# uoguelph-mlrg/Theano-MPI

Measured on NVIDIA H100. Metric: AlexNet-128b BSP seconds per 5120 images (train+comm, device-timed, max over ranks), lower is better.
Workload: dtype bf16; 1 GPU; model=AlexNet, global_batch=128, input=3x227x227, parallelism=dp1, rule=BSP, push_master=False, cuda_graph=True, overlap=True

## Files before the change

theanompi_b200/csrc/api.h:

```cpp
#pragma once
#include <cuda_runtime.h>
#include <stdint.h>
#include <tuple>
#include "common.cuh"

namespace tmpi {

constexpr int kMaxRanks = 8;
constexpr int kMaxCommBlocks = 1024;

struct CommCtx {
  void* arena[kMaxRanks];
  uint32_t* sig[kMaxRanks];
  uint32_t* epoch;
  void* mc_arena;
  int rank, world;
  long long spin_limit;
};

struct FusedArgs {
  CommCtx ctx;
  long long w_off, g_off, u_off, h_off, wire_off;
  const uint8_t* block_group;
  GroupTable tab;
  const float* lr_ptr;
  float mu;
  int nesterov;
  float inv_k;
  long long lo, hi;
  int wire16;
  int pre_reduced;
  int push_master = 1;
};

struct ReduceArgs {
  CommCtx ctx;
  long long src_off, dst_off, h_off;
  const uint8_t* block_group;
  GroupTable tab;
  float scale;
  long long lo, hi;
  int skip_local_groups;
};

void gemm_set_debug(int flags);
void gemm_set_bulk(int mask);
void gemm_rs_configure(int world, const void* const* peer_g , const void* local_g);
void gemm_rs_add_range(const void* c_lo, const void* c_hi, long long blo, long long per);
void gemm_rs_clear();
int gemm_plan_splits(int tiles, int num_kb, int sms);
int gemm_plan_tall(long long M, int nt, int out_bf16, int sms);
std::tuple<int, int, int> gemm_plan_conv(int kind, long long M, int N, int groups, int num_kb, int tall_ok, int sms);
void gemm(const void* A, const void* B, void* C, const float* bias, int M, int N, int K, long long lda, long long ldb, long long ldc,
          int a_mn, int b_mn, int out_bf16, int bias_mode, int relu, float alpha, int bn_hint, int splitk, int f32, cudaStream_t st,
          int accumulate = 0);
void gemm_sgd(const void* A, const void* B, void* W, void* U, void* H, const void* lr_ptr, float lr_mult, float wd, float mu, int nesterov,
              float inv_k, int M, int N, int K, long long lda, long long ldb, long long ldw, int f32, cudaStream_t st);

void conv_fprop(const void* x, const void* w, void* y, const float* bias, int N, int H, int W, int Ctot, int c_off, int Cg, int KH,
                int KW, int Ho, int Wo, int S, int P, int O, long long ldc, int relu, int dgrad, int f32, cudaStream_t st);
void conv_wgrad(const void* dy, const void* x, void* dw, int N, int H, int W, int Ctot, int c_off, int Cg, int KH, int KW, int Ho,
                int Wo, int S, int P, int O, long long ldy, int accumulate, int f32, cudaStream_t st);
void conv_fprop2(const void* x, const void* w0, const void* w1, void* y0, void* y1, const float* bias0, const float* bias1, int N, int H,
                 int W, int Ctot, int c_off0, int c_off1, int Cg, int KH, int KW, int Ho, int Wo, int S, int P, int O, long long ldc,
                 int relu, int dgrad, int f32, cudaStream_t st);
void conv_wgrad2(const void* dy0, const void* dy1, const void* x, void* dw0, void* dw1, int N, int H, int W, int Ctot, int c_off0,
                 int c_off1, int Cg, int KH, int KW, int Ho, int Wo, int S, int P, int O, long long ldy, int accumulate, int f32,
                 cudaStream_t st);

void space_to_depth(const void* x, void* y, int N, int H, int W, int C, int S, int Hs, int Ws, int Cp, int P, int f32, cudaStream_t st);
void s2d_filter(const void* src, void* dst, int O, int KH, int KW, int C, int S, int KHs, int KWs, int Cp, int dir, int f32, cudaStream_t st);
void lrn_fwd(const void* x, void* y, long long rows, int C, int n, float k, float alpha, float beta, int f32, cudaStream_t st);
void lrn_bwd(const void* x, const void* dy, void* dx, long long rows, int C, int n, float k, float alpha, float beta, int f32, cudaStream_t st);
void pool_fwd(const void* x, void* y, void* arg, int N, int H, int W, int C, int Ho, int Wo, int k, int s, int p, int is_max, int f32,
              cudaStream_t st);
void pool_bwd(const void* dy, const void* arg, void* dx, int N, int H, int W, int C, int Ho, int Wo, int k, int s, int p, int is_max, int f32,
              cudaStream_t st);
void dropout_fwd(const void* x, void* y, void* mask, long long n, float p_drop, unsigned long long seed, int layer, const void* step, int f32,
                 cudaStream_t st);
void dropout_bwd(const void* dy, const void* mask, void* dx, long long n, int f32, cudaStream_t st);
void advance_step(void* step, cudaStream_t st);
void softmax_xent(const void* logits, const void* labels, void* dlogits, void* rowstat, void* out3, int B, int C, float weight,
                  float grad_weight, float label_smoothing, int f32, cudaStream_t st);
enum MixMode : int { MIX_NONE = 0, MIX_MIXUP = 1, MIX_CUTMIX = 2 };
struct MixRecord {
  int mode;
  float lam;
  double lam_raw;
  int cy, cx;
  int y0, y1, x0, x1;
  int H, W;
  int pad[4];
};
static_assert(sizeof(MixRecord) == 64, "MixRecord layout is shared with ops/mixup.py");
struct MixParams {
  double alpha, cutmix_alpha;
  double switch_prob, prob;
  unsigned long long seed;
  int rank;
  int H, W;
};
void mix_draw(const MixParams& p, const void* step, void* rec, int n, cudaStream_t st);
void mix_batch(void* x, const void* rec, int B, int H, int W, int C, int f32, cudaStream_t st);
void softmax_xent_mix(const void* logits, const void* labels, const void* rec, void* dlogits, void* rowstat, void* out3, int B, int C,
                      float weight, float grad_weight, float label_smoothing, int f32, cudaStream_t st);
void drop_path_draw(const void* thresh, const void* keep_scale, int L, int B, unsigned long long seed, int rank, const void* step, void* out,
                    cudaStream_t st);
void relu_bias_bwd(const void* dy, const void* y, void* dym, void* db, void* db1, int c_split, long long R, int C, long long ld, int act,
                   float slope, int accumulate, int f32, cudaStream_t st);
void bias_act(const void* acc, const void* bias, void* y, int R, int C, int act, float slope, int f32, cudaStream_t st);
void col2im_bias_act(const void* dcol, void* y, const float* bias, int N, int H, int W, int C, int KH, int KW, int Hi, int Wi, int s, int p,
                     long long ldcol, int act, float slope, int c_real, int f32, cudaStream_t st);
void gan_loss(const void* scores, void* dscores, void* out, int B, int kind, float a, int f32, cudaStream_t st);
void uniform_noise(void* out, long long n, unsigned long long seed, int stream, const void* step, int f32, cudaStream_t st);
void maxpool_relu_bias_bwd(const void* dyp, const void* arg, const void* y, void* dym, void* db0, void* db1, int c_split, int N, int H,
                           int W, int C, int Ho, int Wo, int k, int s, int p, int accumulate, cudaStream_t st);
void im2col(const void* x, void* col, int N, int H, int W, int Ctot, int c_off, int Cg, int KH, int KW, int Ho, int Wo, int s, int p,
            long long ldcol, int f32, cudaStream_t st);
void col2im(const void* dcol, void* dx, int N, int H, int W, int Ctot, int c_off, int Cg, int KH, int KW, int Ho, int Wo, int s, int p,
            long long ldcol, int f32, cudaStream_t st);
void pad_rows(const void* src, void* dst, long long rows, int cols, long long src_ld, long long dst_ld, int f32, cudaStream_t st);
void crop_mirror_norm(const void* x, int in_kind, const void* mean, int mean_mode, float scale, const void* cscale, void* out, int out_bf16, const void* offs,
                      const void* flips, int N, int H, int W, int C, int ch, int cw, int Cout, cudaStream_t st);
void resized_crop_mirror_norm(const void* x, const void* mean, int mean_mode, float scale, const void* cscale, void* out, int out_bf16,
                              const void* boxes, const void* flips, int N, int H, int W, int C, int ch, int cw, cudaStream_t st);

void bn_forward(const void* x, const void* res, void* y, const void* gamma, const void* beta, void* mean, void* rstd, void* run_mean,
                void* run_var, void* scratch, long long R, int C, float momentum, float eps, int training, int act, float slope,
                const void* drop_scale, int batch, int f32, cudaStream_t st);
void bn_backward(const void* x, const void* dy, const void* y, void* dx, void* dres, const void* gamma, const void* mean, const void* rstd,
                 void* dgamma, void* dbeta, void* scratch, long long R, int C, int act, float slope, int accumulate, const void* drop_scale,
                 int batch, int f32, cudaStream_t st);
void add_tensors(const void* a, const void* b, void* y, long long n, int f32, cudaStream_t st);
void add_scaled(const void* a, const void* b, const void* scale, void* y, long long n, int batch, int f32, cudaStream_t st);
void add4_tensors(const void* a, const void* b, const void* c, const void* d, void* y, long long n, int f32, cudaStream_t st);

void lstm_cell_fwd(const void* gx, const void* gh, const void* c_prev, const void* h_prev, const void* mask, void* act, void* c_out, void* h_out,
                   int B, int H, int f32, cudaStream_t st);
void lstm_cell_bwd(const void* dh_out, const void* dh_rec, const void* dh_pass_in, const void* dc_next, const void* act, const void* c,
                   const void* c_prev, const void* mask, void* dG, void* dc_prev, void* dh_pass, int B, int H, int f32, cudaStream_t st);
void embedding_fwd(const void* ids, const void* W, void* out, long long n, int D, int f32, cudaStream_t st);
void embedding_bwd(const void* ids, const void* dout, void* dW, long long n, int D, long long V, int f32, cudaStream_t st);
void masked_mean_fwd(const void* h, const void* mask, void* out, int Tn, int B, int H, int f32, cudaStream_t st);
void masked_mean_bwd(const void* dout, const void* mask, void* dh, int Tn, int B, int H, int f32, cudaStream_t st);

enum FlatRuleId : int { FLAT_SGD = 0, FLAT_ADAM, FLAT_RMSPROP, FLAT_ADADELTA, FLAT_RMSPROP_CENTERED, FLAT_LARS, FLAT_LAMB };
struct ClipRecord {
  float norm;
  float scale;
  int finite;
  int pad;
};
struct FlatUpdateArgs {
  int rule;
  void* W;
  const void* G;
  void* S[3];
  void* H;
  const void* block_group;
  GroupTable tab;
  const void* lr_ptr;
  void* step;
  const float* hp;
  int n_hp;
  long long lo, hi;
  int filter;
  const void* block_tensor;
  const void* tensor_scale;
  const void* clip;
};
void flat_update(const FlatUpdateArgs& a, cudaStream_t st);
struct GradClipArgs {
  const void* G;
  const void* block_tensor;
  const void* tensor_span;
  long long n_blocks;
  float max_norm;
  void* partial;
  void* rec;
  void* skipped;
};
void grad_clip_norm(const GradClipArgs& a, cudaStream_t st);
struct LarsTrustArgs {
  const void* W;
  const void* G;
  const void* block_tensor;
  const void* tensor_span;
  const void* block_group;
  GroupTable tab;
  float inv_k, eta;
  long long n_blocks;
  int n_tensors;
  void* partial;
  void* norms;
  void* trust;
};
void lars_trust(const LarsTrustArgs& a, cudaStream_t st);
struct LambTrustArgs {
  const void* W;
  const void* G;
  void* M;
  void* V;
  const void* step;
  float b1, b2, eps, inv_k;
  int filter;
  const void* block_tensor;
  const void* tensor_span;
  const void* block_group;
  GroupTable tab;
  long long n_blocks;
  int n_tensors;
  void* partial;
  void* norms;
  void* trust;
};
void lamb_trust(const LambTrustArgs& a, cudaStream_t st);
enum LrPolicy : int { LR_CONSTANT = 0, LR_COSINE, LR_POLY, LR_MULTISTEP };
constexpr int kMaxLrMilestones = 8;
struct LrScheduleParams {
  int policy;
  int n_milestones;
  long long warmup, total;
  double start, peak, final_lr, power, gamma;
  long long milestones[kMaxLrMilestones];
};
void lr_schedule(const LrScheduleParams& p, void* counter, void* lr, cudaStream_t st);
void fused_allreduce_sgd(const FusedArgs& a, int algo, int max_blocks, cudaStream_t st);
void push_master_slices(const FusedArgs& a, int max_blocks, cudaStream_t st);
void allreduce_flat(const ReduceArgs& a, int algo, int max_blocks, cudaStream_t st);
void device_barrier(const CommCtx& c, cudaStream_t st);
void easgd_elastic(void* w, void* h, void* center, float alpha, long long n, int max_blocks, int lockfree, cudaStream_t st);
void ticket_acquire(const CommCtx& c, int owner, void* local_state, cudaStream_t st);
void ticket_release(const CommCtx& c, int owner, void* local_state, cudaStream_t st);
void copy_flat(void* dst, void* dst_h, const void* src, long long n, int max_blocks, const void* gate, cudaStream_t st);
void gosgd_push(const CommCtx& c, void* state, int dest, long long w_off, long long snap_off, long long n, int max_blocks, cudaStream_t st);
void gosgd_poll_merge(const CommCtx& c, void* state, long long w_off, long long h_off, long long snap_off, long long n, int max_blocks,
                      cudaStream_t st);
void gosgd_merge(void* w, void* h, const void* b, float a_self, float a_src, long long n, int max_blocks, cudaStream_t st);
void cast_flat(const void* src, void* dst, long long n, int kind, cudaStream_t st);
void sum_chunks(const void* src, void* dst, long long chunk, int nchunks, int is_half, cudaStream_t st);
void vecadd(void* cur, const void* tmp, long long n, int is_half, cudaStream_t st);

}
```

theanompi_b200/csrc/binding.cpp:

```cpp
#include <pybind11/pybind11.h>
#include <pybind11/stl.h>

#include <cstring>
#include <memory>
#include <vector>

#include "api.h"
#include "peer_arena.h"

namespace py = pybind11;
using namespace tmpi;
typedef uintptr_t ptr_t;

static inline void* P(ptr_t p) { return reinterpret_cast<void*>(p); }
static inline cudaStream_t S(ptr_t s) { return reinterpret_cast<cudaStream_t>(s); }

static GroupTable make_table(const std::vector<float>& lr_mult, const std::vector<float>& wd, const std::vector<int>& exch) {
  GroupTable t;
  for (int i = 0; i < kMaxGroups; ++i) {
    t.lr_mult[i] = i < (int)lr_mult.size() ? lr_mult[i] : 1.f;
    t.wd[i] = i < (int)wd.size() ? wd[i] : 0.f;
    t.exch[i] = i < (int)exch.size() ? exch[i] : 1;
  }
  return t;
}

struct PyComm {
  std::unique_ptr<PeerArena> pa;
};

PYBIND11_MODULE(_tmpi_native, m) {
  m.doc() = "theanompi_b200 native sm_90a kernels and peer-memory runtime";
  m.def("launch_count", [] { return (unsigned long long)g_launch_count.load(); });
  m.def("reset_launch_count", [] { g_launch_count.store(0); });
  m.def("capture_status", [](ptr_t st) {
    cudaStreamCaptureStatus s = cudaStreamCaptureStatusNone;
    cudaError_t e = cudaStreamIsCapturing(S(st), &s);
    return py::make_tuple((int)e, (int)s);
  });
  m.attr("ARENA_BLOCK") = kArenaBlock;
  m.attr("MAX_RANKS") = kMaxRanks;
  m.attr("MAX_COMM_BLOCKS") = kMaxCommBlocks;

  m.def("gemm_set_debug", &gemm_set_debug);
  m.def("gemm_set_bulk", &gemm_set_bulk);
  m.def("gemm_rs_add_range", [](ptr_t c_lo, ptr_t c_hi, long long blo, long long per) { gemm_rs_add_range(P(c_lo), P(c_hi), blo, per); });
  m.def("gemm_rs_clear", &gemm_rs_clear);
  m.def("gemm_plan_splits", &gemm_plan_splits);
  m.def("gemm_plan_tall", &gemm_plan_tall);
  m.def("gemm_plan_conv", &gemm_plan_conv);
  m.def("gemm", [](ptr_t A, ptr_t B, ptr_t C, ptr_t bias, int M, int N, int K, long long lda, long long ldb, long long ldc, int a_mn, int b_mn,
                   int out_bf16, int bias_mode, int relu, float alpha, int bn_hint, int splitk, int f32, ptr_t st, int accumulate) {
    gemm(P(A), P(B), P(C), (const float*)P(bias), M, N, K, lda, ldb, ldc, a_mn, b_mn, out_bf16, bias_mode, relu, alpha, bn_hint, splitk, f32,
         S(st), accumulate);
  }, py::arg("A"), py::arg("B"), py::arg("C"), py::arg("bias"), py::arg("M"), py::arg("N"), py::arg("K"), py::arg("lda"), py::arg("ldb"),
     py::arg("ldc"), py::arg("a_mn"), py::arg("b_mn"), py::arg("out_bf16"), py::arg("bias_mode"), py::arg("relu"), py::arg("alpha"),
     py::arg("bn_hint"), py::arg("splitk"), py::arg("f32"), py::arg("st"), py::arg("accumulate") = 0);
  m.def("gemm_sgd", [](ptr_t A, ptr_t B, ptr_t W, ptr_t U, ptr_t H, ptr_t lr_ptr, float lr_mult, float wd, float mu, int nesterov, float inv_k,
                       int M, int N, int K, long long lda, long long ldb, long long ldw, int f32, ptr_t st) {
    gemm_sgd(P(A), P(B), P(W), P(U), P(H), P(lr_ptr), lr_mult, wd, mu, nesterov, inv_k, M, N, K, lda, ldb, ldw, f32, S(st));
  }, py::arg("A"), py::arg("B"), py::arg("W"), py::arg("U"), py::arg("H"), py::arg("lr_ptr"), py::arg("lr_mult"), py::arg("wd"),
     py::arg("mu"), py::arg("nesterov"), py::arg("inv_k"), py::arg("M"), py::arg("N"), py::arg("K"), py::arg("lda"), py::arg("ldb"),
     py::arg("ldw"), py::arg("f32"), py::arg("st"));

  m.def("conv_fprop", [](ptr_t x, ptr_t w, ptr_t y, ptr_t bias, int N, int H, int W, int Ctot, int c_off, int Cg, int KH, int KW, int Ho, int Wo,
                         int Sd, int Pd, int O, long long ldc, int relu, int dgrad, int f32, ptr_t st) {
    conv_fprop(P(x), P(w), P(y), (const float*)P(bias), N, H, W, Ctot, c_off, Cg, KH, KW, Ho, Wo, Sd, Pd, O, ldc, relu, dgrad, f32, S(st)); });
  m.def("conv_wgrad", [](ptr_t dy, ptr_t x, ptr_t dw, int N, int H, int W, int Ctot, int c_off, int Cg, int KH, int KW, int Ho, int Wo, int Sd,
                         int Pd, int O, long long ldy, int accumulate, int f32, ptr_t st) {
    conv_wgrad(P(dy), P(x), P(dw), N, H, W, Ctot, c_off, Cg, KH, KW, Ho, Wo, Sd, Pd, O, ldy, accumulate, f32, S(st)); });
  m.def("conv_fprop2", [](ptr_t x, ptr_t w0, ptr_t w1, ptr_t y0, ptr_t y1, ptr_t b0, ptr_t b1, int N, int H, int W, int Ctot, int c_off0, int c_off1,
                          int Cg, int KH, int KW, int Ho, int Wo, int Sd, int Pd, int O, long long ldc, int relu, int dgrad, int f32, ptr_t st) {
    conv_fprop2(P(x), P(w0), P(w1), P(y0), P(y1), (const float*)P(b0), (const float*)P(b1), N, H, W, Ctot, c_off0, c_off1, Cg, KH, KW, Ho, Wo,
                Sd, Pd, O, ldc, relu, dgrad, f32, S(st)); });
  m.def("conv_wgrad2", [](ptr_t dy0, ptr_t dy1, ptr_t x, ptr_t dw0, ptr_t dw1, int N, int H, int W, int Ctot, int c_off0, int c_off1, int Cg,
                          int KH, int KW, int Ho, int Wo, int Sd, int Pd, int O, long long ldy, int accumulate, int f32, ptr_t st) {
    conv_wgrad2(P(dy0), P(dy1), P(x), P(dw0), P(dw1), N, H, W, Ctot, c_off0, c_off1, Cg, KH, KW, Ho, Wo, Sd, Pd, O, ldy, accumulate, f32,
                S(st)); });
  m.def("space_to_depth", [](ptr_t x, ptr_t y, int N, int H, int W, int C, int Sd, int Hs, int Ws, int Cp, int Pd, int f32, ptr_t st) {
    space_to_depth(P(x), P(y), N, H, W, C, Sd, Hs, Ws, Cp, Pd, f32, S(st)); });
  m.def("s2d_filter", [](ptr_t src, ptr_t dst, int O, int KH, int KW, int C, int Sd, int KHs, int KWs, int Cp, int dir, int f32, ptr_t st) {
    s2d_filter(P(src), P(dst), O, KH, KW, C, Sd, KHs, KWs, Cp, dir, f32, S(st)); });

  m.def("lrn_fwd", [](ptr_t x, ptr_t y, long long rows, int C, int n, float k, float alpha, float beta, int f32, ptr_t st) {
    lrn_fwd(P(x), P(y), rows, C, n, k, alpha, beta, f32, S(st)); });
  m.def("lrn_bwd", [](ptr_t x, ptr_t dy, ptr_t dx, long long rows, int C, int n, float k, float alpha, float beta, int f32, ptr_t st) {
    lrn_bwd(P(x), P(dy), P(dx), rows, C, n, k, alpha, beta, f32, S(st)); });
  m.def("pool_fwd", [](ptr_t x, ptr_t y, ptr_t arg, int N, int H, int W, int C, int Ho, int Wo, int k, int s, int p, int is_max, int f32, ptr_t st) {
    pool_fwd(P(x), P(y), P(arg), N, H, W, C, Ho, Wo, k, s, p, is_max, f32, S(st)); });
  m.def("pool_bwd", [](ptr_t dy, ptr_t arg, ptr_t dx, int N, int H, int W, int C, int Ho, int Wo, int k, int s, int p, int is_max, int f32, ptr_t st) {
    pool_bwd(P(dy), P(arg), P(dx), N, H, W, C, Ho, Wo, k, s, p, is_max, f32, S(st)); });
  m.def("dropout_fwd", [](ptr_t x, ptr_t y, ptr_t mask, long long n, float p, unsigned long long seed, int layer, ptr_t step, int f32, ptr_t st) {
    dropout_fwd(P(x), P(y), P(mask), n, p, seed, layer, P(step), f32, S(st)); });
  m.def("dropout_bwd", [](ptr_t dy, ptr_t mask, ptr_t dx, long long n, int f32, ptr_t st) { dropout_bwd(P(dy), P(mask), P(dx), n, f32, S(st)); });
  m.def("advance_step", [](ptr_t step, ptr_t st) { advance_step(P(step), S(st)); });
  m.def("softmax_xent", [](ptr_t logits, ptr_t labels, ptr_t dlogits, ptr_t rowstat, ptr_t out3, int B, int C, float weight, float grad_weight,
                           float label_smoothing, int f32, ptr_t st) {
    softmax_xent(P(logits), P(labels), P(dlogits), P(rowstat), P(out3), B, C, weight, grad_weight, label_smoothing, f32, S(st)); });
  m.attr("MIX_RECORD_BYTES") = (int)sizeof(MixRecord);
  m.def("mix_draw", [](double alpha, double cutmix_alpha, double switch_prob, double prob, unsigned long long seed, int rank, int H, int W,
                       ptr_t step, ptr_t rec, int n, ptr_t st) {
    mix_draw(MixParams{alpha, cutmix_alpha, switch_prob, prob, seed, rank, H, W}, P(step), P(rec), n, S(st)); });
  m.def("mix_batch", [](ptr_t x, ptr_t rec, int B, int H, int W, int C, int f32, ptr_t st) { mix_batch(P(x), P(rec), B, H, W, C, f32, S(st)); });
  m.def("softmax_xent_mix", [](ptr_t logits, ptr_t labels, ptr_t rec, ptr_t dlogits, ptr_t rowstat, ptr_t out3, int B, int C, float weight,
                               float grad_weight, float label_smoothing, int f32, ptr_t st) {
    softmax_xent_mix(P(logits), P(labels), P(rec), P(dlogits), P(rowstat), P(out3), B, C, weight, grad_weight, label_smoothing, f32, S(st)); });
  m.def("maxpool_relu_bias_bwd", [](ptr_t dyp, ptr_t arg, ptr_t y, ptr_t dym, ptr_t db0, ptr_t db1, int c_split, int N, int H, int W, int C,
                                    int Ho, int Wo, int k, int s, int p, int accumulate, ptr_t st) {
    maxpool_relu_bias_bwd(P(dyp), P(arg), P(y), P(dym), P(db0), P(db1), c_split, N, H, W, C, Ho, Wo, k, s, p, accumulate, S(st)); });
  m.def("relu_bias_bwd", [](ptr_t dy, ptr_t y, ptr_t dym, ptr_t db, ptr_t db1, int c_split, long long R, int C, long long ld, int act, float slope,
                            int accumulate, int f32, ptr_t st) {
    relu_bias_bwd(P(dy), P(y), P(dym), P(db), P(db1), c_split, R, C, ld, act, slope, accumulate, f32, S(st)); });
  m.def("bias_act", [](ptr_t acc, ptr_t bias, ptr_t y, int R, int C, int act, float slope, int f32, ptr_t st) {
    bias_act(P(acc), P(bias), P(y), R, C, act, slope, f32, S(st)); });
  m.def("col2im_bias_act", [](ptr_t dcol, ptr_t y, ptr_t bias, int N, int H, int W, int C, int KH, int KW, int Hi, int Wi, int s, int p,
                              long long ldcol, int act, float slope, int c_real, int f32, ptr_t st) {
    col2im_bias_act(P(dcol), P(y), (const float*)P(bias), N, H, W, C, KH, KW, Hi, Wi, s, p, ldcol, act, slope, c_real, f32, S(st)); });
  m.def("gan_loss", [](ptr_t scores, ptr_t dscores, ptr_t out, int B, int kind, float a, int f32, ptr_t st) {
    gan_loss(P(scores), P(dscores), P(out), B, kind, a, f32, S(st)); });
  m.def("uniform_noise", [](ptr_t out, long long n, unsigned long long seed, int stream, ptr_t step, int f32, ptr_t st) {
    uniform_noise(P(out), n, seed, stream, P(step), f32, S(st)); });
  m.def("im2col", [](ptr_t x, ptr_t col, int N, int H, int W, int Ctot, int c_off, int Cg, int KH, int KW, int Ho, int Wo, int s, int p,
                     long long ldcol, int f32, ptr_t st) { im2col(P(x), P(col), N, H, W, Ctot, c_off, Cg, KH, KW, Ho, Wo, s, p, ldcol, f32, S(st)); });
  m.def("col2im", [](ptr_t dcol, ptr_t dx, int N, int H, int W, int Ctot, int c_off, int Cg, int KH, int KW, int Ho, int Wo, int s, int p,
                     long long ldcol, int f32, ptr_t st) { col2im(P(dcol), P(dx), N, H, W, Ctot, c_off, Cg, KH, KW, Ho, Wo, s, p, ldcol, f32, S(st)); });
  m.def("pad_rows", [](ptr_t src, ptr_t dst, long long rows, int cols, long long src_ld, long long dst_ld, int f32, ptr_t st) {
    pad_rows(P(src), P(dst), rows, cols, src_ld, dst_ld, f32, S(st)); });
  m.def("crop_mirror_norm", [](ptr_t x, int in_kind, ptr_t mean, int mean_mode, float scale, ptr_t cscale, ptr_t out, int out_bf16, ptr_t offs,
                               ptr_t flips, int N, int H, int W, int C, int ch, int cw, int Cout, ptr_t st) {
    crop_mirror_norm(P(x), in_kind, P(mean), mean_mode, scale, P(cscale), P(out), out_bf16, P(offs), P(flips), N, H, W, C, ch, cw, Cout, S(st)); });
  m.def("resized_crop_mirror_norm", [](ptr_t x, ptr_t mean, int mean_mode, float scale, ptr_t cscale, ptr_t out, int out_bf16, ptr_t boxes,
                                       ptr_t flips, int N, int H, int W, int C, int ch, int cw, ptr_t st) {
    resized_crop_mirror_norm(P(x), P(mean), mean_mode, scale, P(cscale), P(out), out_bf16, P(boxes), P(flips), N, H, W, C, ch, cw, S(st)); });

  m.def("bn_forward", [](ptr_t x, ptr_t res, ptr_t y, ptr_t gamma, ptr_t beta, ptr_t mean, ptr_t rstd, ptr_t run_mean, ptr_t run_var, ptr_t scratch,
                         long long R, int C, float momentum, float eps, int training, int act, float slope, ptr_t drop_scale, int batch, int f32,
                         ptr_t st) {
    bn_forward(P(x), P(res), P(y), P(gamma), P(beta), P(mean), P(rstd), P(run_mean), P(run_var), P(scratch), R, C, momentum, eps, training, act,
               slope, P(drop_scale), batch, f32, S(st)); });
  m.def("bn_backward", [](ptr_t x, ptr_t dy, ptr_t y, ptr_t dx, ptr_t dres, ptr_t gamma, ptr_t mean, ptr_t rstd, ptr_t dgamma, ptr_t dbeta,
                          ptr_t scratch, long long R, int C, int act, float slope, int accumulate, ptr_t drop_scale, int batch, int f32, ptr_t st) {
    bn_backward(P(x), P(dy), P(y), P(dx), P(dres), P(gamma), P(mean), P(rstd), P(dgamma), P(dbeta), P(scratch), R, C, act, slope, accumulate,
                P(drop_scale), batch, f32, S(st)); });
  m.def("add_scaled", [](ptr_t a, ptr_t b, ptr_t scale, ptr_t y, long long n, int batch, int f32, ptr_t st) {
    add_scaled(P(a), P(b), P(scale), P(y), n, batch, f32, S(st)); });
  m.def("drop_path_draw", [](ptr_t thresh, ptr_t keep_scale, int L, int B, unsigned long long seed, int rank, ptr_t step, ptr_t out, ptr_t st) {
    drop_path_draw(P(thresh), P(keep_scale), L, B, seed, rank, P(step), P(out), S(st)); });
  m.def("add4_tensors", [](ptr_t a, ptr_t b, ptr_t c, ptr_t d, ptr_t y, long long n, int f32, ptr_t st) {
    add4_tensors(P(a), P(b), P(c), P(d), P(y), n, f32, S(st)); });
  m.def("add_tensors", [](ptr_t a, ptr_t b, ptr_t y, long long n, int f32, ptr_t st) { add_tensors(P(a), P(b), P(y), n, f32, S(st)); });

  m.def("lstm_cell_fwd", [](ptr_t gx, ptr_t gh, ptr_t c_prev, ptr_t h_prev, ptr_t mask, ptr_t act, ptr_t c_out, ptr_t h_out, int B, int H, int f32,
                            ptr_t st) { lstm_cell_fwd(P(gx), P(gh), P(c_prev), P(h_prev), P(mask), P(act), P(c_out), P(h_out), B, H, f32, S(st)); });
  m.def("lstm_cell_bwd", [](ptr_t dh_out, ptr_t dh_rec, ptr_t dh_pass_in, ptr_t dc_next, ptr_t act, ptr_t c, ptr_t c_prev, ptr_t mask, ptr_t dG,
                            ptr_t dc_prev, ptr_t dh_pass, int B, int H, int f32, ptr_t st) {
    lstm_cell_bwd(P(dh_out), P(dh_rec), P(dh_pass_in), P(dc_next), P(act), P(c), P(c_prev), P(mask), P(dG), P(dc_prev), P(dh_pass), B, H, f32, S(st)); });
  m.def("embedding_fwd", [](ptr_t ids, ptr_t W, ptr_t out, long long n, int D, int f32, ptr_t st) { embedding_fwd(P(ids), P(W), P(out), n, D, f32, S(st)); });
  m.def("embedding_bwd", [](ptr_t ids, ptr_t dout, ptr_t dW, long long n, int D, long long V, int f32, ptr_t st) {
    embedding_bwd(P(ids), P(dout), P(dW), n, D, V, f32, S(st)); });
  m.def("masked_mean_fwd", [](ptr_t h, ptr_t mask, ptr_t out, int Tn, int B, int H, int f32, ptr_t st) { masked_mean_fwd(P(h), P(mask), P(out), Tn, B, H, f32, S(st)); });
  m.def("masked_mean_bwd", [](ptr_t dout, ptr_t mask, ptr_t dh, int Tn, int B, int H, int f32, ptr_t st) { masked_mean_bwd(P(dout), P(mask), P(dh), Tn, B, H, f32, S(st)); });

  m.attr("FLAT_RULES") = py::dict(py::arg("sgd") = (int)FLAT_SGD, py::arg("adam") = (int)FLAT_ADAM, py::arg("rmsprop") = (int)FLAT_RMSPROP,
                                   py::arg("adadelta") = (int)FLAT_ADADELTA, py::arg("rmsprop_centered") = (int)FLAT_RMSPROP_CENTERED,
                                   py::arg("lars") = (int)FLAT_LARS, py::arg("lamb") = (int)FLAT_LAMB);
  m.def("flat_update", [](int rule, ptr_t W, ptr_t G, ptr_t S0, ptr_t S1, ptr_t S2, ptr_t H, ptr_t block_group, std::vector<float> lr_mult,
                          std::vector<float> wd, std::vector<int> exch, ptr_t lr_ptr, ptr_t step, std::vector<float> hp, long long lo,
                          long long hi, int filter, ptr_t block_tensor, ptr_t tensor_scale, ptr_t clip, ptr_t st) {
    flat_update(FlatUpdateArgs{rule, P(W), P(G), {P(S0), P(S1), P(S2)}, P(H), P(block_group), make_table(lr_mult, wd, exch), P(lr_ptr),
                               P(step), hp.data(), (int)hp.size(), lo, hi, filter, P(block_tensor), P(tensor_scale), P(clip)}, S(st)); });
  m.def("grad_clip_norm", [](ptr_t G, ptr_t block_tensor, ptr_t tensor_span, long long n_blocks, float max_norm, ptr_t partial, ptr_t rec,
                             ptr_t skipped, ptr_t st) {
    grad_clip_norm(GradClipArgs{P(G), P(block_tensor), P(tensor_span), n_blocks, max_norm, P(partial), P(rec), P(skipped)}, S(st)); });
  m.def("lars_trust", [](ptr_t W, ptr_t G, ptr_t block_tensor, ptr_t tensor_span, ptr_t block_group, std::vector<float> lr_mult,
                         std::vector<float> wd, std::vector<int> exch, float inv_k, float eta, long long n_blocks, int n_tensors,
                         ptr_t partial, ptr_t norms, ptr_t trust, ptr_t st) {
    lars_trust(LarsTrustArgs{P(W), P(G), P(block_tensor), P(tensor_span), P(block_group), make_table(lr_mult, wd, exch), inv_k, eta,
                             n_blocks, n_tensors, P(partial), P(norms), P(trust)}, S(st)); });
  m.def("lamb_trust", [](ptr_t W, ptr_t G, ptr_t M, ptr_t V, ptr_t step, float b1, float b2, float eps, float inv_k, int filter,
                         ptr_t block_tensor, ptr_t tensor_span, ptr_t block_group, std::vector<float> lr_mult, std::vector<float> wd,
                         std::vector<int> exch, long long n_blocks, int n_tensors, ptr_t partial, ptr_t norms, ptr_t trust, ptr_t st) {
    lamb_trust(LambTrustArgs{P(W), P(G), P(M), P(V), P(step), b1, b2, eps, inv_k, filter, P(block_tensor), P(tensor_span), P(block_group),
                             make_table(lr_mult, wd, exch), n_blocks, n_tensors, P(partial), P(norms), P(trust)}, S(st)); });
  m.attr("LR_POLICIES") = py::dict(py::arg("constant") = (int)LR_CONSTANT, py::arg("cosine") = (int)LR_COSINE,
                                    py::arg("poly") = (int)LR_POLY, py::arg("multistep") = (int)LR_MULTISTEP);
  m.def("lr_schedule", [](int policy, long long warmup, long long total, double start, double peak, double final_lr, double power,
                          double gamma, std::vector<long long> milestones, ptr_t counter, ptr_t lr, ptr_t st) {
    if (milestones.size() > (size_t)kMaxLrMilestones) throw std::runtime_error("lr_schedule: at most 8 milestones");
    LrScheduleParams p{};
    p.policy = policy; p.n_milestones = (int)milestones.size(); p.warmup = warmup; p.total = total;
    p.start = start; p.peak = peak; p.final_lr = final_lr; p.power = power; p.gamma = gamma;
    for (size_t k = 0; k < milestones.size(); ++k) p.milestones[k] = milestones[k];
    lr_schedule(p, P(counter), P(lr), S(st));
  });
  m.def("easgd_elastic", [](ptr_t w, ptr_t h, ptr_t center, float alpha, long long n, int max_blocks, ptr_t st, int lockfree) {
    easgd_elastic(P(w), P(h), P(center), alpha, n, max_blocks, lockfree, S(st)); },
    py::arg("w"), py::arg("h"), py::arg("center"), py::arg("alpha"), py::arg("n"), py::arg("max_blocks"), py::arg("st"), py::arg("lockfree") = 0);
  m.def("copy_flat", [](ptr_t dst, ptr_t dst_h, ptr_t src, long long n, int max_blocks, ptr_t st) {
    copy_flat(P(dst), P(dst_h), P(src), n, max_blocks, nullptr, S(st)); });
  m.def("gosgd_merge", [](ptr_t w, ptr_t h, ptr_t b, float a_self, float a_src, long long n, int max_blocks, ptr_t st) {
    gosgd_merge(P(w), P(h), P(b), a_self, a_src, n, max_blocks, S(st)); });
  m.def("cast_flat", [](ptr_t src, ptr_t dst, long long n, int kind, ptr_t st) { cast_flat(P(src), P(dst), n, kind, S(st)); });
  m.def("sum_chunks", [](ptr_t src, ptr_t dst, long long chunk, int nchunks, int is_half, ptr_t st) {
    sum_chunks(P(src), P(dst), chunk, nchunks, is_half, S(st)); });
  m.def("vecadd", [](ptr_t cur, ptr_t tmp, long long n, int is_half, ptr_t st) { vecadd(P(cur), P(tmp), n, is_half, S(st)); });

  py::class_<PyComm, std::shared_ptr<PyComm>>(m, "PeerArena")
      .def(py::init([](int rank, int world, int device, unsigned long long bytes, const std::string& job, bool force_ipc) {
        auto c = std::make_shared<PyComm>();
        c->pa.reset(new PeerArena(rank, world, device, (size_t)bytes, job, force_ipc));
        return c;
      }), py::arg("rank"), py::arg("world"), py::arg("device"), py::arg("bytes"), py::arg("job"), py::arg("force_ipc") = false)
      .def("send_handles_to", [](PyComm& c, int peer) { py::gil_scoped_release r; c.pa->send_handles_to(peer); })
      .def("recv_handles", [](PyComm& c) { py::gil_scoped_release r; c.pa->recv_handles(); })
      .def("ipc_handles", [](PyComm& c) { return py::bytes(c.pa->ipc_handles()); })
      .def("ipc_open", [](PyComm& c, int peer, const std::string& h) { c.pa->ipc_open(peer, h); })
      .def("multicast_supported", [](PyComm& c) { return c.pa->multicast_supported(); })
      .def("mc_create_and_send", [](PyComm& c) { py::gil_scoped_release r; c.pa->mc_create_and_send(); })
      .def("mc_recv", [](PyComm& c) { py::gil_scoped_release r; c.pa->mc_recv(); })
      .def("mc_add_device", [](PyComm& c) { c.pa->mc_add_device(); })
      .def("mc_bind_and_map", [](PyComm& c) { c.pa->mc_bind_and_map(); })
      .def("arena_ptr", [](PyComm& c, int p) { return (ptr_t)c.pa->arena_ptr(p); })
      .def("sig_ptr", [](PyComm& c, int p) { return (ptr_t)c.pa->sig_ptr(p); })
      .def("mc_ptr", [](PyComm& c) { return (ptr_t)c.pa->mc_ptr(); })
      .def("arena_bytes", [](PyComm& c) { return (unsigned long long)c.pa->arena_bytes(); })
      .def("mode", [](PyComm& c) { return c.pa->mode(); })
      .def("vmm_error", [](PyComm& c) { return c.pa->vmm_error(); })
      .def("device_barrier", [](PyComm& c, ptr_t st) { device_barrier(c.pa->ctx(), S(st)); })
      .def("ticket_acquire", [](PyComm& c, int owner, ptr_t local_state, ptr_t st) { ticket_acquire(c.pa->ctx(), owner, P(local_state), S(st)); })
      .def("ticket_release", [](PyComm& c, int owner, ptr_t local_state, ptr_t st) { ticket_release(c.pa->ctx(), owner, P(local_state), S(st)); })
      .def("gosgd_push", [](PyComm& c, ptr_t state, int dest, long long w_off, long long snap_off, long long n, int max_blocks, ptr_t st) {
             gosgd_push(c.pa->ctx(), P(state), dest, w_off, snap_off, n, max_blocks, S(st)); })
      .def("gosgd_poll_merge", [](PyComm& c, ptr_t state, long long w_off, long long h_off, long long snap_off, long long n, int max_blocks,
                                  ptr_t st) { gosgd_poll_merge(c.pa->ctx(), P(state), w_off, h_off, snap_off, n, max_blocks, S(st)); })
      .def("proto_words_offset", [](PyComm&) { return (long long)((size_t)kMaxCommBlocks * kMaxRanks + kMaxCommBlocks) * 4; })
      .def("fused_allreduce_sgd",
           [](PyComm& c, long long w_off, long long g_off, long long u_off, long long h_off, long long wire_off, ptr_t block_group,
              std::vector<float> lr_mult, std::vector<float> wd, std::vector<int> exch, ptr_t lr_ptr, float mu, int nesterov, float inv_k,
              long long lo, long long hi, int wire16, int algo, int max_blocks, ptr_t st, int pre_reduced, int push_master) {
             FusedArgs a;
             a.pre_reduced = pre_reduced;
             a.push_master = push_master;
             a.ctx = c.pa->ctx();
             a.w_off = w_off; a.g_off = g_off; a.u_off = u_off; a.h_off = h_off; a.wire_off = wire_off;
             a.block_group = (const uint8_t*)P(block_group);
             a.tab = make_table(lr_mult, wd, exch);
             a.lr_ptr = (const float*)P(lr_ptr); a.mu = mu; a.nesterov = nesterov; a.inv_k = inv_k; a.lo = lo; a.hi = hi; a.wire16 = wire16;
             fused_allreduce_sgd(a, algo, max_blocks, S(st));
           }, py::arg("w_off"), py::arg("g_off"), py::arg("u_off"), py::arg("h_off"), py::arg("wire_off"), py::arg("block_group"),
           py::arg("lr_mult"), py::arg("wd"), py::arg("exch"), py::arg("lr_ptr"), py::arg("mu"), py::arg("nesterov"), py::arg("inv_k"),
           py::arg("lo"), py::arg("hi"), py::arg("wire16"), py::arg("algo"), py::arg("max_blocks"), py::arg("st"), py::arg("pre_reduced") = 0,
           py::arg("push_master") = 1)
      .def("push_master_slices",
           [](PyComm& c, long long w_off, ptr_t block_group, std::vector<float> lr_mult, std::vector<float> wd, std::vector<int> exch,
              long long lo, long long hi, int max_blocks, ptr_t st) {
             FusedArgs a;
             a.pre_reduced = 0; a.ctx = c.pa->ctx();
             a.w_off = w_off; a.g_off = a.u_off = a.wire_off = 0; a.h_off = -1;
             a.block_group = (const uint8_t*)P(block_group);
             a.tab = make_table(lr_mult, wd, exch);
             a.lr_ptr = nullptr; a.mu = 0.f; a.nesterov = 0; a.inv_k = 1.f; a.lo = lo; a.hi = hi; a.wire16 = 0;
             push_master_slices(a, max_blocks, S(st));
           })
      .def("configure_gemm_rs", [](PyComm& c, long long g_off) {
             const CommCtx x = c.pa->ctx();
             const void* peers[kMaxRanks];
             for (int p = 0; p < x.world; ++p) peers[p] = reinterpret_cast<const char*>(x.arena[p]) + g_off;
             gemm_rs_configure(x.world, peers, peers[x.rank]);
           })
      .def("allreduce_flat",
           [](PyComm& c, long long src_off, long long dst_off, long long h_off, ptr_t block_group, std::vector<float> lr_mult,
              std::vector<float> wd, std::vector<int> exch, float scale, long long lo, long long hi, int skip_local, int algo,
              int max_blocks, ptr_t st) {
             ReduceArgs a;
             a.ctx = c.pa->ctx();
             a.src_off = src_off; a.dst_off = dst_off; a.h_off = h_off;
             a.block_group = (const uint8_t*)P(block_group);
             a.tab = make_table(lr_mult, wd, exch);
             a.scale = scale; a.lo = lo; a.hi = hi; a.skip_local_groups = skip_local;
             allreduce_flat(a, algo, max_blocks, S(st));
           });
}
```

theanompi_b200/csrc/gemm_wgmma.cu:

```cuda
#include "gemm_wgmma.cuh"
#include <vector>

namespace tmpi {
std::atomic<unsigned long long> g_launch_count{0};

namespace wgmma {

int g_dbg = 0;
int g_bulk = -1;

static int choose_splits(int tiles, int num_kb, int sms) {
  if (deterministic_mode()) return 1;
  if (tiles >= sms || num_kb < 8) return 1;
  const int kTileOverheadKb = 4;
  int best = 1;
  long long best_cost = -1;
  const int max_s = std::min(num_kb / 4, 4 * sms);
  for (int s = 1; s <= max_s; ++s) {
    const int kb_per = (num_kb + s - 1) / s;
    const int s_eff = (num_kb + kb_per - 1) / kb_per;
    const long long waves = ((long long)tiles * s_eff + sms - 1) / sms;
    const long long cost = waves * (kb_per + kTileOverheadKb) * 64 + s_eff;
    if (best_cost < 0 || cost < best_cost) { best_cost = cost; best = s_eff; }
  }
  return best;
}

static bool use_tall_tiles(long long M, int nt, int eligible, int sms) {
  static const bool enabled = [] { const char* e = getenv("TMPI_GEMM_TALL"); return !(e && e[0] == '0'); }();
  if (!enabled || !eligible || M < 2 * BM) return false;
  const long long t1 = ((M + BM - 1) / BM) * nt, t2 = ((M + 2 * BM - 1) / (2 * BM)) * nt;
  const long long w1 = (t1 + sms - 1) / sms, w2 = (t2 + sms - 1) / sms;
  return w2 * 17 <= w1 * 10;
}

struct ConvTile { int bn, mt, splits; };
static ConvTile choose_conv_tile(int kind, long long M, int N, int groups, int num_kb, int tall_ok, int sms) {
  static const int kCand[7][2] = {{128, 2}, {128, 1}, {192, 1}, {96, 2}, {96, 1}, {64, 2}, {64, 1}};
  const int kTileOverheadKb = 4, kKblockCols = 64;
  const int kWideWgradMinKb = 1024;
  ConvTile best{0, 0, 1};
  long long best_cost = -1;
  for (const auto& c : kCand) {
    const int bn = c[0], mt = c[1];
    if (bn == 96 && kind != 0) continue;
    if (kind == 2 && (bn == 64 || mt == 2)) continue;
    if (kind == 2 && bn == 192 && num_kb < kWideWgradMinKb) continue;
    const int nt = (N + bn - 1) / bn;
    if (mt == 2 && !use_tall_tiles(M, nt * groups, tall_ok, sms)) continue;
    const long long tiles = ((M + mt * BM - 1) / (mt * BM)) * nt * groups;
    int splits = kind == 2 ? choose_splits((int)tiles, num_kb, sms) : 1;
    const int kb_per = (num_kb + splits - 1) / splits;
    splits = (num_kb + kb_per - 1) / kb_per;
    const long long waves = (tiles * splits + sms - 1) / sms;
    const long long cost = waves * (kb_per + kTileOverheadKb) * (mt * bn + kKblockCols);
    if (best_cost < 0 || cost < best_cost) { best_cost = cost; best = {bn, mt, splits}; }
  }
  return best;
}

}

void gemm_set_debug(int flags) { wgmma::g_dbg = flags; }
void gemm_set_bulk(int mask) { wgmma::g_bulk = mask; }

namespace wgmma {
struct RsRange { const char* lo; const char* hi; long long blo, per; };
static int g_rs_world = 0, g_rs_rank = 0;
static float* g_rs_peer[kMaxRanks] = {};
static const char* g_rs_local = nullptr;
static std::vector<RsRange> g_rs_ranges;
static std::mutex g_rs_mu;
static bool rs_lookup(const void* C, Params& p) {
  std::lock_guard<std::mutex> lk(g_rs_mu);
  if (g_rs_world < 2) return false;
  const char* c = reinterpret_cast<const char*>(C);
  for (const RsRange& r : g_rs_ranges) {
    if (c >= r.lo && c < r.hi) {
      p.rs_world = g_rs_world; p.rs_rank = g_rs_rank;
      p.rs_blo = (unsigned)r.blo; p.rs_per = (unsigned)std::max<long long>(1, r.per);
      p.rs_e0 = (long long)((c - g_rs_local) / 4);
      for (int q = 0; q < kMaxRanks; ++q) p.rs_g[q] = q < g_rs_world ? g_rs_peer[q] : nullptr;
      return true;
    }
  }
  return false;
}
}

void gemm_rs_configure(int world, const void* const* peer_g, const void* local_g) {
  std::lock_guard<std::mutex> lk(wgmma::g_rs_mu);
  if (world > kMaxRanks) throw std::runtime_error("gemm_rs_configure: too many ranks");
  wgmma::g_rs_world = world;
  wgmma::g_rs_local = reinterpret_cast<const char*>(local_g);
  wgmma::g_rs_rank = 0;
  for (int q = 0; q < world; ++q) {
    wgmma::g_rs_peer[q] = reinterpret_cast<float*>(const_cast<void*>(peer_g[q]));
    if (peer_g[q] == local_g) wgmma::g_rs_rank = q;
  }
  wgmma::g_rs_ranges.clear();
}
void gemm_rs_add_range(const void* c_lo, const void* c_hi, long long blo, long long per) {
  std::lock_guard<std::mutex> lk(wgmma::g_rs_mu);
  wgmma::g_rs_ranges.push_back({reinterpret_cast<const char*>(c_lo), reinterpret_cast<const char*>(c_hi), blo, per});
}
void gemm_rs_clear() {
  std::lock_guard<std::mutex> lk(wgmma::g_rs_mu);
  wgmma::g_rs_world = 0; wgmma::g_rs_ranges.clear();
}

int gemm_plan_splits(int tiles, int num_kb, int sms) { return wgmma::choose_splits(tiles, num_kb, sms); }
int gemm_plan_tall(long long M, int nt, int out_bf16, int sms) { return wgmma::use_tall_tiles(M, nt, out_bf16, sms) ? 1 : 0; }
std::tuple<int, int, int> gemm_plan_conv(int kind, long long M, int N, int groups, int num_kb, int tall_ok, int sms) {
  const wgmma::ConvTile t = wgmma::choose_conv_tile(kind, M, N, groups, num_kb, tall_ok, sms);
  return {t.bn, t.mt, t.splits};
}

namespace wgmma {
template <typename T>
static void gemm_host(const void* A, const void* B, void* C, const float* bias, int M, int N, int K, long long lda, long long ldb,
                      long long ldc, int a_mn, int b_mn, int out_bf16, int bias_mode, int relu, float alpha, int bn_hint, int splitk,
                      int accumulate, cudaStream_t st) {
  using E = Elem<T>;
  constexpr int BK = E::BK, ATOM = E::ATOM, ESZ = E::ESZ;
  if (M <= 0 || N <= 0 || K <= 0) return;
  const int sms = sm_count();
  const int mt = (M + BM - 1) / BM;
  const bool fused_epi = bias_mode != 0 || relu;
  const bool can_split = (!out_bf16) && !fused_epi;
  if (accumulate && !can_split) throw std::runtime_error("gemm: accumulate needs an fp32 output without bias / ReLU");
  int BN = bn_hint;
  if (BN == 0) {
    BN = 128;
    if (!(can_split && splitk != 1)) {
      if (mt * ((N + 127) / 128) < sms && N >= 64) BN = 64;
      if (BN == 64 && mt * ((N + 63) / 64) < sms && !b_mn && N >= 32) BN = 32;
    } else if (N <= 64) {
      BN = 64;
    }
  }
  if (b_mn && BN < 64) BN = 64;
  const int nt = (N + BN - 1) / BN;
  const int num_kb = (K + BK - 1) / BK;
  int splits = 1;
  if (splitk > 1 && can_split) splits = splitk;
  else if (splitk == 0 && can_split) splits = choose_splits(mt * nt, num_kb, sms);
  int kb_per = (num_kb + splits - 1) / splits;
  splits = (num_kb + kb_per - 1) / kb_per;

  Params p;
  p.C = C; p.bias = bias; p.alpha = alpha; p.M = M; p.N = N; p.K = K; p.ldc = ldc; p.a_mn = a_mn; p.b_mn = b_mn;
  p.out_bf16 = out_bf16; p.bias_mode = bias ? bias_mode : 0; p.relu = relu; p.kb_per_split = kb_per; p.atomic_out = splits > 1 || accumulate;
  const int tall_ok = ESZ == 2 ? out_bf16 : (!a_mn && !b_mn);
  const bool tall = splits == 1 && BN >= 64 && use_tall_tiles(M, nt, tall_ok, sms);
  p.mt = tall ? (M + 2 * BM - 1) / (2 * BM) : mt; p.nt = nt; p.splits = splits; p.num_kb = num_kb; p.conv_mode = 0;
  p.group_m = (p.mt > 12 && nt > 12) ? (tall ? 8 : 12) : 0;
  p.cHo = p.cWo = p.cS = p.cP = p.cKH = p.cKW = p.cCg = p.c_chunks = 0;
  const bool rs = !accumulate && (!out_bf16) && bias_mode == 0 && !relu && alpha == 1.f && (ldc % 4) == 0 && rs_lookup(C, p);
  if (rs) {
    p.atomic_out = 1;
  } else if (splits > 1 && !accumulate) {
    check_cuda(cudaMemset2DAsync(C, (size_t)ldc * 4, 0, (size_t)N * 4, (size_t)M, st), "gemm split-K memset");
  }
  CUtensorMap ta = a_mn ? make_tmap(A, (uint64_t)M, (uint64_t)K, (uint64_t)lda * ESZ, (uint32_t)BK, ESZ, 1)
                        : make_tmap(A, (uint64_t)K, (uint64_t)M, (uint64_t)lda * ESZ, (uint32_t)BM, ESZ, 0);
  CUtensorMap tb = b_mn ? make_tmap(B, (uint64_t)N, (uint64_t)K, (uint64_t)ldb * ESZ, (uint32_t)BK, ESZ, 1)
                        : make_tmap(B, (uint64_t)K, (uint64_t)N, (uint64_t)ldb * ESZ, (uint32_t)BN, ESZ, 0);
  (void)ATOM;
  if (tall) { if (BN == 128) launch<T, 128, 2>(ta, tb, p, splits, st); else launch<T, 64, 2>(ta, tb, p, splits, st); }
  else if (BN == 128) launch<T, 128, 1>(ta, tb, p, splits, st);
  else if (BN == 64) launch<T, 64, 1>(ta, tb, p, splits, st);
  else launch<T, 32, 1>(ta, tb, p, splits, st);
}
}

void gemm(const void* A, const void* B, void* C, const float* bias, int M, int N, int K, long long lda, long long ldb,
          long long ldc, int a_mn, int b_mn, int out_bf16, int bias_mode, int relu, float alpha, int bn_hint, int splitk, int f32,
          cudaStream_t st, int accumulate) {
  if (f32) wgmma::gemm_host<float>(A, B, C, bias, M, N, K, lda, ldb, ldc, a_mn, b_mn, 0, bias_mode, relu, alpha, bn_hint, splitk, accumulate, st);
  else wgmma::gemm_host<__nv_bfloat16>(A, B, C, bias, M, N, K, lda, ldb, ldc, a_mn, b_mn, out_bf16, bias_mode, relu, alpha, bn_hint, splitk,
                                       accumulate, st);
}

namespace wgmma {
typedef CUresult (*PFN_encodeIm2col)(CUtensorMap*, CUtensorMapDataType, cuuint32_t, void*, const cuuint64_t*, const cuuint64_t*, const int*,
                                     const int*, cuuint32_t, cuuint32_t, const cuuint32_t*, CUtensorMapInterleave, CUtensorMapSwizzle,
                                     CUtensorMapL2promotion, CUtensorMapFloatOOBfill);
static PFN_encodeIm2col get_encode_im2col() {
  static PFN_encodeIm2col fn = nullptr;
  static std::once_flag once;
  std::call_once(once, [] {
    void* f = nullptr;
    cudaDriverEntryPointQueryResult q;
    if (cudaGetDriverEntryPoint("cuTensorMapEncodeIm2col", &f, cudaEnableDefault, &q) == cudaSuccess && q == cudaDriverEntryPointSuccess)
      fn = (PFN_encodeIm2col)f;
    (void)cudaGetLastError();
  });
  if (!fn) throw std::runtime_error("tmpi_native: cuTensorMapEncodeIm2col unavailable");
  return fn;
}

static CUtensorMap make_im2col_map(const void* x, int N, int H, int W, int Ctot, int c_off, int Cg, int KH, int KW, int S, int P, int pixels,
                                   int esz, int mn_major) {
  const char* base = reinterpret_cast<const char*>(x) + (size_t)c_off * esz;
  if ((reinterpret_cast<uintptr_t>(base) & 15) != 0 || ((Ctot * esz) % 16) != 0) throw std::runtime_error("tmpi_native: im2col operand must be 16B aligned");
  using Key = std::tuple<const void*, int, int, int, int, int, int, int, int, int, int, int, int>;
  static std::map<Key, CUtensorMap> cache;
  static std::mutex mu;
  Key key{base, N, H, W, Ctot, Cg, KH, KW, S, P, pixels, esz, mn_major};
  const CUtensorMapSwizzle swz = CU_TENSOR_MAP_SWIZZLE_128B;
  std::lock_guard<std::mutex> lk(mu);
  auto it = cache.find(key);
  if (it != cache.end()) return it->second;
  CUtensorMap m;
  cuuint64_t dims[4] = {(cuuint64_t)Cg, (cuuint64_t)W, (cuuint64_t)H, (cuuint64_t)N};
  cuuint64_t strides[3] = {(cuuint64_t)Ctot * esz, (cuuint64_t)W * Ctot * esz, (cuuint64_t)H * W * Ctot * esz};
  int lower[2] = {-P, -P};
  int upper[2] = {P - (KW - 1), P - (KH - 1)};
  cuuint32_t estr[4] = {1u, (cuuint32_t)S, (cuuint32_t)S, 1u};
  CUresult r = get_encode_im2col()(&m, esz == 4 ? f32_map_type() : CU_TENSOR_MAP_DATA_TYPE_BFLOAT16, 4, const_cast<char*>(base),
                                   dims, strides, lower, upper, (cuuint32_t)(128 / esz), (cuuint32_t)pixels, estr,
                                   CU_TENSOR_MAP_INTERLEAVE_NONE, swz, CU_TENSOR_MAP_L2_PROMOTION_L2_256B,
                                   CU_TENSOR_MAP_FLOAT_OOB_FILL_NONE);
  if (r != CUDA_SUCCESS) throw std::runtime_error("tmpi_native: cuTensorMapEncodeIm2col failed, code " + std::to_string((int)r));
  if (cache.size() > 4096) cache.clear();
  cache[key] = m;
  return m;
}

static CUtensorMap make_weight_map(const void* w, int O, int taps, int Cg, int box_o, int box_c, int esz, int mn_major) {
  if ((reinterpret_cast<uintptr_t>(w) & 15) != 0 || ((Cg * esz) % 16) != 0) throw std::runtime_error("tmpi_native: conv weights must be 16B aligned, C * esz % 16 == 0");
  using Key = std::tuple<const void*, int, int, int, int, int, int, int>;
  static std::map<Key, CUtensorMap> cache;
  static std::mutex mu;
  Key key{w, O, taps, Cg, box_o, box_c, esz, mn_major};
  const CUtensorMapSwizzle swz = CU_TENSOR_MAP_SWIZZLE_128B;
  std::lock_guard<std::mutex> lk(mu);
  auto it = cache.find(key);
  if (it != cache.end()) return it->second;
  CUtensorMap m;
  cuuint64_t dims[3] = {(cuuint64_t)Cg, (cuuint64_t)taps, (cuuint64_t)O};
  cuuint64_t strides[2] = {(cuuint64_t)Cg * esz, (cuuint64_t)taps * Cg * esz};
  cuuint32_t box[3] = {(cuuint32_t)box_c, 1u, (cuuint32_t)box_o};
  cuuint32_t estr[3] = {1u, 1u, 1u};
  CUresult r = get_encode()(&m, esz == 4 ? f32_map_type() : CU_TENSOR_MAP_DATA_TYPE_BFLOAT16, 3, const_cast<void*>(w), dims, strides,
                            box, estr, CU_TENSOR_MAP_INTERLEAVE_NONE, swz, CU_TENSOR_MAP_L2_PROMOTION_L2_256B,
                            CU_TENSOR_MAP_FLOAT_OOB_FILL_NONE);
  if (r != CUDA_SUCCESS) throw std::runtime_error("tmpi_native: cuTensorMapEncodeTiled(3D weights) failed, code " + std::to_string((int)r));
  if (cache.size() > 4096) cache.clear();
  cache[key] = m;
  return m;
}

template <typename T>
static void conv_fprop_groups(int ngroups, const void* x, const int* c_off, const void* const* w, void* const* y, const float* const* bias,
                              int N, int H, int W, int Ctot, int Cg, int KH, int KW, int Ho, int Wo, int S, int P, int O, long long ldc,
                              int relu, int out_bf16, int dgrad, cudaStream_t st) {
  using E = Elem<T>;
  constexpr int BK = E::BK, ATOM = E::ATOM, ESZ = E::ESZ;
  const long long M = (long long)N * Ho * Wo;
  if (M <= 0 || O <= 0) return;
  if (M >= (1LL << 31)) throw std::runtime_error("conv_fprop: too many output pixels");
  if (ESZ == 4) out_bf16 = 0;
  const int c_chunks = (Cg + BK - 1) / BK, num_kb = KH * KW * c_chunks;
  const ConvTile tile = choose_conv_tile(dgrad ? 1 : 0, M, O, ngroups, num_kb, ESZ == 2 ? out_bf16 : !dgrad, sm_count());
  const int BN = tile.bn;
  const bool tall = tile.mt == 2;
  Params p;
  p.C = y[0]; p.bias = bias[0]; p.alpha = 1.f; p.M = (int)M; p.N = O; p.K = KH * KW * Cg; p.ldc = ldc; p.a_mn = 0; p.b_mn = dgrad ? 1 : 0;
  p.groups = ngroups; p.C1 = ngroups > 1 ? y[1] : nullptr; p.bias1 = ngroups > 1 ? bias[1] : nullptr;
  p.out_bf16 = out_bf16; p.bias_mode = bias[0] ? 1 : 0; p.relu = relu; p.atomic_out = 0;
  if (ngroups > 1 && ((bias[0] == nullptr) != (bias[1] == nullptr))) throw std::runtime_error("conv_fprop: both groups need a bias or none");
  if (dgrad && (S != 1 || ((O * ESZ) % 16) != 0)) throw std::runtime_error("conv dgrad through the fprop kernel needs stride 1 and 16-byte channel rows");
  p.nt = (O + BN - 1) / BN; p.splits = 1;
  p.mt = tall ? (int)((M + 2 * BM - 1) / (2 * BM)) : (int)((M + BM - 1) / BM);
  p.group_m = 0;
  p.conv_mode = 1; p.cHo = Ho; p.cWo = Wo; p.cS = S; p.cP = P; p.cKH = KH; p.cKW = KW; p.cCg = Cg; p.c_chunks = c_chunks;
  p.num_kb = num_kb; p.kb_per_split = p.num_kb;
  CUtensorMap ta[2], tb[2];
  for (int g = 0; g < ngroups; ++g) {
    ta[g] = make_im2col_map(x, N, H, W, Ctot, c_off[g], Cg, KH, KW, S, P, BM, ESZ, 0);
    tb[g] = dgrad ? make_weight_map(w[g], Cg, KH * KW, O, BK, ATOM, ESZ, 1) : make_weight_map(w[g], O, KH * KW, Cg, BN, BK, ESZ, 0);
  }
  const CUtensorMap* a1 = ngroups > 1 ? &ta[1] : nullptr;
  const CUtensorMap* b1 = ngroups > 1 ? &tb[1] : nullptr;
  if (tall) {
    if (BN == 128) launch<T, 128, 2>(ta[0], tb[0], p, 1, st, a1, b1);
    else if (BN == 96) launch<T, 96, 2>(ta[0], tb[0], p, 1, st, a1, b1);
    else launch<T, 64, 2>(ta[0], tb[0], p, 1, st, a1, b1);
  } else if (BN == 192) launch<T, 192, 1>(ta[0], tb[0], p, 1, st, a1, b1);
  else if (BN == 128) launch<T, 128, 1>(ta[0], tb[0], p, 1, st, a1, b1);
  else if (BN == 96) launch<T, 96, 1>(ta[0], tb[0], p, 1, st, a1, b1);
  else launch<T, 64, 1>(ta[0], tb[0], p, 1, st, a1, b1);
}

template <typename T>
static void conv_wgrad_groups(int ngroups, const void* const* dy, const void* x, void* const* dw, const int* c_off, int N, int H, int W,
                              int Ctot, int Cg, int KH, int KW, int Ho, int Wo, int S, int P, int O, long long ldy, int accumulate,
                              cudaStream_t st) {
  using E = Elem<T>;
  constexpr int BK = E::BK, ATOM = E::ATOM, ESZ = E::ESZ;
  const long long M = (long long)N * Ho * Wo;
  if (M <= 0 || O <= 0) return;
  if (M >= (1LL << 31)) throw std::runtime_error("conv_wgrad: too many output pixels");
  const int c_chunks = (Cg + ATOM - 1) / ATOM, num_kb = (int)((M + BK - 1) / BK);
  const ConvTile tile = choose_conv_tile(2, O, KH * KW * c_chunks * ATOM, ngroups, num_kb, 0, sm_count());
  const int BN = tile.bn;
  Params p;
  p.C = dw[0]; p.bias = nullptr; p.alpha = 1.f; p.M = O; p.N = KH * KW * Cg; p.K = (int)M; p.ldc = (long long)KH * KW * Cg; p.a_mn = 1; p.b_mn = 1;
  p.groups = ngroups; p.C1 = ngroups > 1 ? dw[1] : nullptr; p.bias1 = nullptr;
  p.out_bf16 = 0; p.bias_mode = 0; p.relu = 0;
  p.group_m = 0;
  p.conv_mode = 2; p.cHo = Ho; p.cWo = Wo; p.cS = S; p.cP = P; p.cKH = KH; p.cKW = KW; p.cCg = Cg; p.c_chunks = c_chunks;
  p.mt = (O + BM - 1) / BM; p.nt = (KH * KW * p.c_chunks + BN / ATOM - 1) / (BN / ATOM);
  p.num_kb = num_kb;
  const int splits = tile.splits;
  p.kb_per_split = (p.num_kb + splits - 1) / splits;
  p.splits = splits; p.atomic_out = splits > 1 || accumulate;
  CUtensorMap ta[2], tb[2];
  for (int g = 0; g < ngroups; ++g) {
    if (splits > 1 && !accumulate) check_cuda(cudaMemsetAsync(dw[g], 0, (size_t)O * KH * KW * Cg * 4, st), "conv_wgrad memset");
    ta[g] = make_tmap(dy[g], (uint64_t)O, (uint64_t)M, (uint64_t)ldy * ESZ, (uint32_t)BK, ESZ, 1);
    tb[g] = make_im2col_map(x, N, H, W, Ctot, c_off[g], Cg, KH, KW, S, P, BK, ESZ, 1);
  }
  const CUtensorMap* a1 = ngroups > 1 ? &ta[1] : nullptr;
  const CUtensorMap* b1 = ngroups > 1 ? &tb[1] : nullptr;
  if (BN == 192) launch<T, 192, 1>(ta[0], tb[0], p, splits, st, a1, b1);
  else launch<T, 128, 1>(ta[0], tb[0], p, splits, st, a1, b1);
}
}

void conv_fprop(const void* x, const void* w, void* y, const float* bias, int N, int H, int W, int Ctot, int c_off, int Cg, int KH,
                int KW, int Ho, int Wo, int S, int P, int O, long long ldc, int relu, int dgrad, int f32, cudaStream_t st) {
  const void* ws[1] = {w}; void* ys[1] = {y}; const float* bs[1] = {bias};
  if (f32) wgmma::conv_fprop_groups<float>(1, x, &c_off, ws, ys, bs, N, H, W, Ctot, Cg, KH, KW, Ho, Wo, S, P, O, ldc, relu, 0, dgrad, st);
  else wgmma::conv_fprop_groups<__nv_bfloat16>(1, x, &c_off, ws, ys, bs, N, H, W, Ctot, Cg, KH, KW, Ho, Wo, S, P, O, ldc, relu, 1, dgrad, st);
}

void conv_fprop2(const void* x, const void* w0, const void* w1, void* y0, void* y1, const float* bias0, const float* bias1, int N, int H,
                 int W, int Ctot, int c_off0, int c_off1, int Cg, int KH, int KW, int Ho, int Wo, int S, int P, int O, long long ldc,
                 int relu, int dgrad, int f32, cudaStream_t st) {
  const int co[2] = {c_off0, c_off1}; const void* ws[2] = {w0, w1}; void* ys[2] = {y0, y1}; const float* bs[2] = {bias0, bias1};
  if (f32) wgmma::conv_fprop_groups<float>(2, x, co, ws, ys, bs, N, H, W, Ctot, Cg, KH, KW, Ho, Wo, S, P, O, ldc, relu, 0, dgrad, st);
  else wgmma::conv_fprop_groups<__nv_bfloat16>(2, x, co, ws, ys, bs, N, H, W, Ctot, Cg, KH, KW, Ho, Wo, S, P, O, ldc, relu, 1, dgrad, st);
}

void conv_wgrad(const void* dy, const void* x, void* dw, int N, int H, int W, int Ctot, int c_off, int Cg, int KH, int KW, int Ho,
                int Wo, int S, int P, int O, long long ldy, int accumulate, int f32, cudaStream_t st) {
  const void* dys[1] = {dy}; void* dws[1] = {dw};
  if (f32) wgmma::conv_wgrad_groups<float>(1, dys, x, dws, &c_off, N, H, W, Ctot, Cg, KH, KW, Ho, Wo, S, P, O, ldy, accumulate, st);
  else wgmma::conv_wgrad_groups<__nv_bfloat16>(1, dys, x, dws, &c_off, N, H, W, Ctot, Cg, KH, KW, Ho, Wo, S, P, O, ldy, accumulate, st);
}

void conv_wgrad2(const void* dy0, const void* dy1, const void* x, void* dw0, void* dw1, int N, int H, int W, int Ctot, int c_off0,
                 int c_off1, int Cg, int KH, int KW, int Ho, int Wo, int S, int P, int O, long long ldy, int accumulate, int f32,
                 cudaStream_t st) {
  const void* dys[2] = {dy0, dy1}; void* dws[2] = {dw0, dw1}; const int co[2] = {c_off0, c_off1};
  if (f32) wgmma::conv_wgrad_groups<float>(2, dys, x, dws, co, N, H, W, Ctot, Cg, KH, KW, Ho, Wo, S, P, O, ldy, accumulate, st);
  else wgmma::conv_wgrad_groups<__nv_bfloat16>(2, dys, x, dws, co, N, H, W, Ctot, Cg, KH, KW, Ho, Wo, S, P, O, ldy, accumulate, st);
}

}
```

theanompi_b200/csrc/gemm_wgmma.cuh:

```cuda
#pragma once
#include "common.cuh"
#include "api.h"
#include <cuda.h>
#include <algorithm>
#include <map>
#include <mutex>
#include <tuple>

namespace tmpi {

namespace wgmma {

constexpr int BM = 128;
constexpr int NUM_THREADS = 384;
constexpr int NUM_CONSUMER_WARPS = 8;
constexpr int PRODUCER_REGS = 40, CONSUMER_REGS = 232;

template <typename T> struct SgdEpilogue {};
template <typename OP> struct Operand { using Type = OP; static constexpr bool kSgd = false; };
template <typename T> struct Operand<SgdEpilogue<T>> { using Type = T; static constexpr bool kSgd = true; };

template <typename T> struct Elem {
  static constexpr int ESZ = (int)sizeof(T);
  static constexpr int BK = 128 / ESZ;
  static constexpr int MMA_K = 32 / ESZ;
  static constexpr int ATOM = 128 / ESZ;
  static constexpr bool TF32 = ESZ == 4;
};

template <typename T, int BN, int MT> struct Cfg {
  static constexpr int A_BYTES = MT * BM * 128;
  static constexpr int B_BYTES = BN * 128;
  static constexpr int STAGE_BYTES = A_BYTES + B_BYTES;
  static constexpr int STAGING_ROW = 32 * 4 + 16;
  static constexpr int STAGING_BYTES = NUM_CONSUMER_WARPS * 16 * STAGING_ROW;
  static constexpr bool XPOSE = Elem<T>::TF32 && MT == 1;
  static constexpr int XA_BYTES = 64 * 128;
  static constexpr int XPOSE_BYTES = XPOSE ? 2 * (XA_BYTES + B_BYTES) : 0;
  static constexpr int SMEM_LIMIT = 232448;
  static constexpr int RING_BUDGET = SMEM_LIMIT - STAGING_BYTES - XPOSE_BYTES - 1024  - 256 ;
  static constexpr int STAGES = (RING_BUDGET / STAGE_BYTES) > 8 ? 8 : (RING_BUDGET / STAGE_BYTES);
  static constexpr int SMEM_BYTES = STAGES * STAGE_BYTES + XPOSE_BYTES + STAGING_BYTES + 1024 + 256;
  static_assert(STAGES >= 3, "operand ring too shallow");
};

struct Params {
  void* C;
  const float* bias;
  float alpha;
  int M, N, K;
  long long ldc;
  int a_mn, b_mn;
  int out_bf16;
  int bias_mode;
  int relu;
  int kb_per_split;
  int mt, nt, splits;
  int num_kb;
  int conv_mode;
  int cHo, cWo, cS, cP, cKH, cKW, cCg, c_chunks;
  int atomic_out;
  void* C1;
  const float* bias1;
  int groups;
  int group_m;
  int dbg;
  int rs_world = 0, rs_rank = 0;
  unsigned rs_blo = 0, rs_per = 1;
  long long rs_e0 = 0;
  float* rs_g[kMaxRanks] = {nullptr, nullptr, nullptr, nullptr, nullptr, nullptr, nullptr, nullptr};
  int bulk = 0;
  struct Sgd {
    float* W = nullptr;
    float* U = nullptr;
    __nv_bfloat16* H = nullptr;
    const float* lr_ptr = nullptr;
    float lr_mult = 1.f, wd = 0.f, mu = 0.f, inv_k = 1.f;
    int nesterov = 0;
    long long ldw = 0;
  } sgd;
};

__device__ __forceinline__ float* rs_addr(const Params& p, long long e, bool& local) {
  unsigned owner = ((unsigned)(e >> 10) - p.rs_blo) / p.rs_per;
  if (owner >= (unsigned)p.rs_world) owner = (unsigned)p.rs_world - 1u;
  float* base = p.rs_g[0];
#pragma unroll
  for (int q = 1; q < kMaxRanks; ++q) if (owner == (unsigned)q) base = p.rs_g[q];
  local = owner == (unsigned)p.rs_rank;
  return base + e;
}
__device__ __forceinline__ void red_add_sys_f32(float* addr, float v) {
  asm volatile("red.relaxed.sys.global.add.f32 [%0], %1;" ::"l"(addr), "f"(v) : "memory");
}

__device__ __forceinline__ uint32_t smem_u32(const void* p) { return (uint32_t)__cvta_generic_to_shared(p); }

__device__ __forceinline__ void mbar_init(uint32_t bar, uint32_t count) {
  asm volatile("mbarrier.init.shared::cta.b64 [%0], %1;" ::"r"(bar), "r"(count));
}
__device__ __forceinline__ void mbar_expect_tx(uint32_t bar, uint32_t bytes) {
  asm volatile("mbarrier.arrive.expect_tx.shared::cta.b64 _, [%0], %1;" ::"r"(bar), "r"(bytes) : "memory");
}
__device__ __forceinline__ void mbar_arrive(uint32_t bar) {
  asm volatile("mbarrier.arrive.shared::cta.b64 _, [%0];" ::"r"(bar) : "memory");
}
__device__ __forceinline__ void mbar_wait(uint32_t bar, uint32_t parity) {
  asm volatile(
      "{\n\t"
      ".reg .pred P1, P2;\n\t"
      ".reg .u32 cnt;\n\t"
      "mov.u32 cnt, 0;\n\t"
      "LAB_WAIT:\n\t"
      "mbarrier.try_wait.parity.shared::cta.b64 P1, [%0], %1;\n\t"
      "@P1 bra DONE;\n\t"
      "add.u32 cnt, cnt, 1;\n\t"
      "setp.lt.u32 P2, cnt, 0x10000000;\n\t"
      "@P2 bra LAB_WAIT;\n\t"
      "trap;\n\t"
      "DONE:\n\t"
      "}"
      ::"r"(bar), "r"(parity) : "memory");
}
__device__ __forceinline__ void fence_barrier_init() { asm volatile("fence.mbarrier_init.release.cluster;" ::: "memory"); }
__device__ __forceinline__ void fence_proxy_async() { asm volatile("fence.proxy.async.shared::cta;" ::: "memory"); }
template <int ID> __device__ __forceinline__ void bar_sync_128() { asm volatile("bar.sync %0, 128;" ::"n"(ID) : "memory"); }
__device__ __forceinline__ void wg_bar(int cw) { if (cw == 0) bar_sync_128<1>(); else bar_sync_128<2>(); }

__device__ __forceinline__ void tma_load_2d(uint32_t dst, const CUtensorMap* map, uint32_t bar, int c0, int c1) {
  asm volatile(
      "cp.async.bulk.tensor.2d.shared::cluster.global.mbarrier::complete_tx::bytes [%0], [%1, {%3, %4}], [%2];"
      ::"r"(dst), "l"(map), "r"(bar), "r"(c0), "r"(c1) : "memory");
}
__device__ __forceinline__ void tma_load_3d(uint32_t dst, const CUtensorMap* map, uint32_t bar, int c0, int c1, int c2) {
  asm volatile(
      "cp.async.bulk.tensor.3d.shared::cluster.global.mbarrier::complete_tx::bytes [%0], [%1, {%3, %4, %5}], [%2];"
      ::"r"(dst), "l"(map), "r"(bar), "r"(c0), "r"(c1), "r"(c2) : "memory");
}
__device__ __forceinline__ void tma_load_im2col(uint32_t dst, const CUtensorMap* map, uint32_t bar, int c, int w, int h, int n,
                                                int off_w, int off_h) {
  asm volatile(
      "cp.async.bulk.tensor.4d.shared::cluster.global.im2col.mbarrier::complete_tx::bytes [%0], [%1, {%3, %4, %5, %6}], [%2], {%7, %8};"
      ::"r"(dst), "l"(map), "r"(bar), "r"(c), "r"(w), "r"(h), "r"(n), "h"((uint16_t)off_w), "h"((uint16_t)off_h) : "memory");
}
__device__ __forceinline__ void bulk_store(void* gdst, uint32_t ssrc, uint32_t bytes) {
  asm volatile("cp.async.bulk.global.shared::cta.bulk_group [%0], [%1], %2;" ::"l"(gdst), "r"(ssrc), "r"(bytes) : "memory");
}
__device__ __forceinline__ void bulk_reduce_add_f32(void* gdst, uint32_t ssrc, uint32_t bytes) {
  asm volatile("cp.reduce.async.bulk.global.shared::cta.bulk_group.add.f32 [%0], [%1], %2;" ::"l"(gdst), "r"(ssrc), "r"(bytes) : "memory");
}
__device__ __forceinline__ void bulk_commit() { asm volatile("cp.async.bulk.commit_group;" ::: "memory"); }
__device__ __forceinline__ void bulk_wait_read() { asm volatile("cp.async.bulk.wait_group.read 0;" ::: "memory"); }
__device__ __forceinline__ void bulk_wait_all() { asm volatile("cp.async.bulk.wait_group 0;" ::: "memory"); }

__device__ __forceinline__ void tma_prefetch_desc(const CUtensorMap* map) {
  asm volatile("prefetch.tensormap [%0];" ::"l"(map) : "memory");
}

__device__ __forceinline__ bool elect_one() {
  uint32_t pred;
  asm volatile(
      "{\n\t.reg .pred P;\n\t"
      "elect.sync _|P, 0xffffffff;\n\t"
      "selp.b32 %0, 1, 0, P;\n\t}"
      : "=r"(pred));
  return pred != 0;
}

__device__ __forceinline__ void wgmma_fence() { asm volatile("wgmma.fence.sync.aligned;" ::: "memory"); }
__device__ __forceinline__ void wgmma_commit() { asm volatile("wgmma.commit_group.sync.aligned;" ::: "memory"); }
__device__ __forceinline__ void wgmma_wait0() { asm volatile("wgmma.wait_group.sync.aligned 0;" ::: "memory"); }
template <int N> __device__ __forceinline__ void acc_fence(float (&d)[N]) {
#pragma unroll
  for (int i = 0; i < N; ++i) asm volatile("" : "+f"(d[i])::"memory");
}

template <int N, int TA, int TB> struct WgBF16 {};
template <int N> struct WgTF32 {};

template <int TA, int TB>
__device__ __forceinline__ void wgmma(float (&d)[16], uint64_t da, uint64_t db, uint32_t scale_d, WgBF16<32, TA, TB>) {
  asm volatile("{\n\t.reg .pred p;\n\tsetp.ne.b32 p, %18, 0;\n\t"
               "wgmma.mma_async.sync.aligned.m64n32k16.f32.bf16.bf16 {%0, %1, %2, %3, %4, %5, %6, %7, %8, %9, %10, %11, %12, %13, %14, %15}, %16, %17, p, 1, 1, %19, %20;\n\t}"
               : "+f"(d[0]), "+f"(d[1]), "+f"(d[2]), "+f"(d[3]), "+f"(d[4]), "+f"(d[5]), "+f"(d[6]), "+f"(d[7]), "+f"(d[8]), "+f"(d[9]), "+f"(d[10]), "+f"(d[11]), "+f"(d[12]), "+f"(d[13]), "+f"(d[14]), "+f"(d[15])
               : "l"(da), "l"(db), "r"(scale_d), "n"(TA), "n"(TB));
}

template <int TA, int TB>
__device__ __forceinline__ void wgmma(float (&d)[32], uint64_t da, uint64_t db, uint32_t scale_d, WgBF16<64, TA, TB>) {
  asm volatile("{\n\t.reg .pred p;\n\tsetp.ne.b32 p, %34, 0;\n\t"
               "wgmma.mma_async.sync.aligned.m64n64k16.f32.bf16.bf16 {%0, %1, %2, %3, %4, %5, %6, %7, %8, %9, %10, %11, %12, %13, %14, %15, %16, %17, %18, %19, %20, %21, %22, %23, %24, %25, %26, %27, %28, %29, %30, %31}, %32, %33, p, 1, 1, %35, %36;\n\t}"
               : "+f"(d[0]), "+f"(d[1]), "+f"(d[2]), "+f"(d[3]), "+f"(d[4]), "+f"(d[5]), "+f"(d[6]), "+f"(d[7]), "+f"(d[8]), "+f"(d[9]), "+f"(d[10]), "+f"(d[11]), "+f"(d[12]), "+f"(d[13]), "+f"(d[14]), "+f"(d[15]), "+f"(d[16]), "+f"(d[17]), "+f"(d[18]), "+f"(d[19]), "+f"(d[20]), "+f"(d[21]), "+f"(d[22]), "+f"(d[23]), "+f"(d[24]), "+f"(d[25]), "+f"(d[26]), "+f"(d[27]), "+f"(d[28]), "+f"(d[29]), "+f"(d[30]), "+f"(d[31])
               : "l"(da), "l"(db), "r"(scale_d), "n"(TA), "n"(TB));
}

template <int TA, int TB>
__device__ __forceinline__ void wgmma(float (&d)[64], uint64_t da, uint64_t db, uint32_t scale_d, WgBF16<128, TA, TB>) {
  asm volatile("{\n\t.reg .pred p;\n\tsetp.ne.b32 p, %66, 0;\n\t"
               "wgmma.mma_async.sync.aligned.m64n128k16.f32.bf16.bf16 {%0, %1, %2, %3, %4, %5, %6, %7, %8, %9, %10, %11, %12, %13, %14, %15, %16, %17, %18, %19, %20, %21, %22, %23, %24, %25, %26, %27, %28, %29, %30, %31, %32, %33, %34, %35, %36, %37, %38, %39, %40, %41, %42, %43, %44, %45, %46, %47, %48, %49, %50, %51, %52, %53, %54, %55, %56, %57, %58, %59, %60, %61, %62, %63}, %64, %65, p, 1, 1, %67, %68;\n\t}"
               : "+f"(d[0]), "+f"(d[1]), "+f"(d[2]), "+f"(d[3]), "+f"(d[4]), "+f"(d[5]), "+f"(d[6]), "+f"(d[7]), "+f"(d[8]), "+f"(d[9]), "+f"(d[10]), "+f"(d[11]), "+f"(d[12]), "+f"(d[13]), "+f"(d[14]), "+f"(d[15]), "+f"(d[16]), "+f"(d[17]), "+f"(d[18]), "+f"(d[19]), "+f"(d[20]), "+f"(d[21]), "+f"(d[22]), "+f"(d[23]), "+f"(d[24]), "+f"(d[25]), "+f"(d[26]), "+f"(d[27]), "+f"(d[28]), "+f"(d[29]), "+f"(d[30]), "+f"(d[31]), "+f"(d[32]), "+f"(d[33]), "+f"(d[34]), "+f"(d[35]), "+f"(d[36]), "+f"(d[37]), "+f"(d[38]), "+f"(d[39]), "+f"(d[40]), "+f"(d[41]), "+f"(d[42]), "+f"(d[43]), "+f"(d[44]), "+f"(d[45]), "+f"(d[46]), "+f"(d[47]), "+f"(d[48]), "+f"(d[49]), "+f"(d[50]), "+f"(d[51]), "+f"(d[52]), "+f"(d[53]), "+f"(d[54]), "+f"(d[55]), "+f"(d[56]), "+f"(d[57]), "+f"(d[58]), "+f"(d[59]), "+f"(d[60]), "+f"(d[61]), "+f"(d[62]), "+f"(d[63])
               : "l"(da), "l"(db), "r"(scale_d), "n"(TA), "n"(TB));
}

__device__ __forceinline__ void wgmma(float (&d)[16], uint64_t da, uint64_t db, uint32_t scale_d, WgTF32<32>) {
  asm volatile("{\n\t.reg .pred p;\n\tsetp.ne.b32 p, %18, 0;\n\t"
               "wgmma.mma_async.sync.aligned.m64n32k8.f32.tf32.tf32 {%0, %1, %2, %3, %4, %5, %6, %7, %8, %9, %10, %11, %12, %13, %14, %15}, %16, %17, p, 1, 1;\n\t}"
               : "+f"(d[0]), "+f"(d[1]), "+f"(d[2]), "+f"(d[3]), "+f"(d[4]), "+f"(d[5]), "+f"(d[6]), "+f"(d[7]), "+f"(d[8]), "+f"(d[9]), "+f"(d[10]), "+f"(d[11]), "+f"(d[12]), "+f"(d[13]), "+f"(d[14]), "+f"(d[15])
               : "l"(da), "l"(db), "r"(scale_d));
}

__device__ __forceinline__ void wgmma(float (&d)[32], uint64_t da, uint64_t db, uint32_t scale_d, WgTF32<64>) {
  asm volatile("{\n\t.reg .pred p;\n\tsetp.ne.b32 p, %34, 0;\n\t"
               "wgmma.mma_async.sync.aligned.m64n64k8.f32.tf32.tf32 {%0, %1, %2, %3, %4, %5, %6, %7, %8, %9, %10, %11, %12, %13, %14, %15, %16, %17, %18, %19, %20, %21, %22, %23, %24, %25, %26, %27, %28, %29, %30, %31}, %32, %33, p, 1, 1;\n\t}"
               : "+f"(d[0]), "+f"(d[1]), "+f"(d[2]), "+f"(d[3]), "+f"(d[4]), "+f"(d[5]), "+f"(d[6]), "+f"(d[7]), "+f"(d[8]), "+f"(d[9]), "+f"(d[10]), "+f"(d[11]), "+f"(d[12]), "+f"(d[13]), "+f"(d[14]), "+f"(d[15]), "+f"(d[16]), "+f"(d[17]), "+f"(d[18]), "+f"(d[19]), "+f"(d[20]), "+f"(d[21]), "+f"(d[22]), "+f"(d[23]), "+f"(d[24]), "+f"(d[25]), "+f"(d[26]), "+f"(d[27]), "+f"(d[28]), "+f"(d[29]), "+f"(d[30]), "+f"(d[31])
               : "l"(da), "l"(db), "r"(scale_d));
}

__device__ __forceinline__ void wgmma(float (&d)[64], uint64_t da, uint64_t db, uint32_t scale_d, WgTF32<128>) {
  asm volatile("{\n\t.reg .pred p;\n\tsetp.ne.b32 p, %66, 0;\n\t"
               "wgmma.mma_async.sync.aligned.m64n128k8.f32.tf32.tf32 {%0, %1, %2, %3, %4, %5, %6, %7, %8, %9, %10, %11, %12, %13, %14, %15, %16, %17, %18, %19, %20, %21, %22, %23, %24, %25, %26, %27, %28, %29, %30, %31, %32, %33, %34, %35, %36, %37, %38, %39, %40, %41, %42, %43, %44, %45, %46, %47, %48, %49, %50, %51, %52, %53, %54, %55, %56, %57, %58, %59, %60, %61, %62, %63}, %64, %65, p, 1, 1;\n\t}"
               : "+f"(d[0]), "+f"(d[1]), "+f"(d[2]), "+f"(d[3]), "+f"(d[4]), "+f"(d[5]), "+f"(d[6]), "+f"(d[7]), "+f"(d[8]), "+f"(d[9]), "+f"(d[10]), "+f"(d[11]), "+f"(d[12]), "+f"(d[13]), "+f"(d[14]), "+f"(d[15]), "+f"(d[16]), "+f"(d[17]), "+f"(d[18]), "+f"(d[19]), "+f"(d[20]), "+f"(d[21]), "+f"(d[22]), "+f"(d[23]), "+f"(d[24]), "+f"(d[25]), "+f"(d[26]), "+f"(d[27]), "+f"(d[28]), "+f"(d[29]), "+f"(d[30]), "+f"(d[31]), "+f"(d[32]), "+f"(d[33]), "+f"(d[34]), "+f"(d[35]), "+f"(d[36]), "+f"(d[37]), "+f"(d[38]), "+f"(d[39]), "+f"(d[40]), "+f"(d[41]), "+f"(d[42]), "+f"(d[43]), "+f"(d[44]), "+f"(d[45]), "+f"(d[46]), "+f"(d[47]), "+f"(d[48]), "+f"(d[49]), "+f"(d[50]), "+f"(d[51]), "+f"(d[52]), "+f"(d[53]), "+f"(d[54]), "+f"(d[55]), "+f"(d[56]), "+f"(d[57]), "+f"(d[58]), "+f"(d[59]), "+f"(d[60]), "+f"(d[61]), "+f"(d[62]), "+f"(d[63])
               : "l"(da), "l"(db), "r"(scale_d));
}

template <int TA, int TB>
__device__ __forceinline__ void wgmma(float (&d)[48], uint64_t da, uint64_t db, uint32_t scale_d, WgBF16<96, TA, TB>) {
  asm volatile("{\n\t.reg .pred p;\n\tsetp.ne.b32 p, %50, 0;\n\t"
               "wgmma.mma_async.sync.aligned.m64n96k16.f32.bf16.bf16 {%0, %1, %2, %3, %4, %5, %6, %7, %8, %9, %10, %11, %12, %13, %14, %15, %16, %17, %18, %19, %20, %21, %22, %23, %24, %25, %26, %27, %28, %29, %30, %31, %32, %33, %34, %35, %36, %37, %38, %39, %40, %41, %42, %43, %44, %45, %46, %47}, %48, %49, p, 1, 1, %51, %52;\n\t}"
               : "+f"(d[0]), "+f"(d[1]), "+f"(d[2]), "+f"(d[3]), "+f"(d[4]), "+f"(d[5]), "+f"(d[6]), "+f"(d[7]), "+f"(d[8]), "+f"(d[9]), "+f"(d[10]), "+f"(d[11]), "+f"(d[12]), "+f"(d[13]), "+f"(d[14]), "+f"(d[15]), "+f"(d[16]), "+f"(d[17]), "+f"(d[18]), "+f"(d[19]), "+f"(d[20]), "+f"(d[21]), "+f"(d[22]), "+f"(d[23]), "+f"(d[24]), "+f"(d[25]), "+f"(d[26]), "+f"(d[27]), "+f"(d[28]), "+f"(d[29]), "+f"(d[30]), "+f"(d[31]), "+f"(d[32]), "+f"(d[33]), "+f"(d[34]), "+f"(d[35]), "+f"(d[36]), "+f"(d[37]), "+f"(d[38]), "+f"(d[39]), "+f"(d[40]), "+f"(d[41]), "+f"(d[42]), "+f"(d[43]), "+f"(d[44]), "+f"(d[45]), "+f"(d[46]), "+f"(d[47])
               : "l"(da), "l"(db), "r"(scale_d), "n"(TA), "n"(TB));
}

template <int TA, int TB>
__device__ __forceinline__ void wgmma(float (&d)[96], uint64_t da, uint64_t db, uint32_t scale_d, WgBF16<192, TA, TB>) {
  asm volatile("{\n\t.reg .pred p;\n\tsetp.ne.b32 p, %98, 0;\n\t"
               "wgmma.mma_async.sync.aligned.m64n192k16.f32.bf16.bf16 {%0, %1, %2, %3, %4, %5, %6, %7, %8, %9, %10, %11, %12, %13, %14, %15, %16, %17, %18, %19, %20, %21, %22, %23, %24, %25, %26, %27, %28, %29, %30, %31, %32, %33, %34, %35, %36, %37, %38, %39, %40, %41, %42, %43, %44, %45, %46, %47, %48, %49, %50, %51, %52, %53, %54, %55, %56, %57, %58, %59, %60, %61, %62, %63, %64, %65, %66, %67, %68, %69, %70, %71, %72, %73, %74, %75, %76, %77, %78, %79, %80, %81, %82, %83, %84, %85, %86, %87, %88, %89, %90, %91, %92, %93, %94, %95}, %96, %97, p, 1, 1, %99, %100;\n\t}"
               : "+f"(d[0]), "+f"(d[1]), "+f"(d[2]), "+f"(d[3]), "+f"(d[4]), "+f"(d[5]), "+f"(d[6]), "+f"(d[7]), "+f"(d[8]), "+f"(d[9]), "+f"(d[10]), "+f"(d[11]), "+f"(d[12]), "+f"(d[13]), "+f"(d[14]), "+f"(d[15]), "+f"(d[16]), "+f"(d[17]), "+f"(d[18]), "+f"(d[19]), "+f"(d[20]), "+f"(d[21]), "+f"(d[22]), "+f"(d[23]), "+f"(d[24]), "+f"(d[25]), "+f"(d[26]), "+f"(d[27]), "+f"(d[28]), "+f"(d[29]), "+f"(d[30]), "+f"(d[31]), "+f"(d[32]), "+f"(d[33]), "+f"(d[34]), "+f"(d[35]), "+f"(d[36]), "+f"(d[37]), "+f"(d[38]), "+f"(d[39]), "+f"(d[40]), "+f"(d[41]), "+f"(d[42]), "+f"(d[43]), "+f"(d[44]), "+f"(d[45]), "+f"(d[46]), "+f"(d[47]), "+f"(d[48]), "+f"(d[49]), "+f"(d[50]), "+f"(d[51]), "+f"(d[52]), "+f"(d[53]), "+f"(d[54]), "+f"(d[55]), "+f"(d[56]), "+f"(d[57]), "+f"(d[58]), "+f"(d[59]), "+f"(d[60]), "+f"(d[61]), "+f"(d[62]), "+f"(d[63]), "+f"(d[64]), "+f"(d[65]), "+f"(d[66]), "+f"(d[67]), "+f"(d[68]), "+f"(d[69]), "+f"(d[70]), "+f"(d[71]), "+f"(d[72]), "+f"(d[73]), "+f"(d[74]), "+f"(d[75]), "+f"(d[76]), "+f"(d[77]), "+f"(d[78]), "+f"(d[79]), "+f"(d[80]), "+f"(d[81]), "+f"(d[82]), "+f"(d[83]), "+f"(d[84]), "+f"(d[85]), "+f"(d[86]), "+f"(d[87]), "+f"(d[88]), "+f"(d[89]), "+f"(d[90]), "+f"(d[91]), "+f"(d[92]), "+f"(d[93]), "+f"(d[94]), "+f"(d[95])
               : "l"(da), "l"(db), "r"(scale_d), "n"(TA), "n"(TB));
}

__device__ __forceinline__ void wgmma(float (&d)[48], uint64_t da, uint64_t db, uint32_t scale_d, WgTF32<96>) {
  asm volatile("{\n\t.reg .pred p;\n\tsetp.ne.b32 p, %50, 0;\n\t"
               "wgmma.mma_async.sync.aligned.m64n96k8.f32.tf32.tf32 {%0, %1, %2, %3, %4, %5, %6, %7, %8, %9, %10, %11, %12, %13, %14, %15, %16, %17, %18, %19, %20, %21, %22, %23, %24, %25, %26, %27, %28, %29, %30, %31, %32, %33, %34, %35, %36, %37, %38, %39, %40, %41, %42, %43, %44, %45, %46, %47}, %48, %49, p, 1, 1;\n\t}"
               : "+f"(d[0]), "+f"(d[1]), "+f"(d[2]), "+f"(d[3]), "+f"(d[4]), "+f"(d[5]), "+f"(d[6]), "+f"(d[7]), "+f"(d[8]), "+f"(d[9]), "+f"(d[10]), "+f"(d[11]), "+f"(d[12]), "+f"(d[13]), "+f"(d[14]), "+f"(d[15]), "+f"(d[16]), "+f"(d[17]), "+f"(d[18]), "+f"(d[19]), "+f"(d[20]), "+f"(d[21]), "+f"(d[22]), "+f"(d[23]), "+f"(d[24]), "+f"(d[25]), "+f"(d[26]), "+f"(d[27]), "+f"(d[28]), "+f"(d[29]), "+f"(d[30]), "+f"(d[31]), "+f"(d[32]), "+f"(d[33]), "+f"(d[34]), "+f"(d[35]), "+f"(d[36]), "+f"(d[37]), "+f"(d[38]), "+f"(d[39]), "+f"(d[40]), "+f"(d[41]), "+f"(d[42]), "+f"(d[43]), "+f"(d[44]), "+f"(d[45]), "+f"(d[46]), "+f"(d[47])
               : "l"(da), "l"(db), "r"(scale_d));
}

__device__ __forceinline__ void wgmma(float (&d)[96], uint64_t da, uint64_t db, uint32_t scale_d, WgTF32<192>) {
  asm volatile("{\n\t.reg .pred p;\n\tsetp.ne.b32 p, %98, 0;\n\t"
               "wgmma.mma_async.sync.aligned.m64n192k8.f32.tf32.tf32 {%0, %1, %2, %3, %4, %5, %6, %7, %8, %9, %10, %11, %12, %13, %14, %15, %16, %17, %18, %19, %20, %21, %22, %23, %24, %25, %26, %27, %28, %29, %30, %31, %32, %33, %34, %35, %36, %37, %38, %39, %40, %41, %42, %43, %44, %45, %46, %47, %48, %49, %50, %51, %52, %53, %54, %55, %56, %57, %58, %59, %60, %61, %62, %63, %64, %65, %66, %67, %68, %69, %70, %71, %72, %73, %74, %75, %76, %77, %78, %79, %80, %81, %82, %83, %84, %85, %86, %87, %88, %89, %90, %91, %92, %93, %94, %95}, %96, %97, p, 1, 1;\n\t}"
               : "+f"(d[0]), "+f"(d[1]), "+f"(d[2]), "+f"(d[3]), "+f"(d[4]), "+f"(d[5]), "+f"(d[6]), "+f"(d[7]), "+f"(d[8]), "+f"(d[9]), "+f"(d[10]), "+f"(d[11]), "+f"(d[12]), "+f"(d[13]), "+f"(d[14]), "+f"(d[15]), "+f"(d[16]), "+f"(d[17]), "+f"(d[18]), "+f"(d[19]), "+f"(d[20]), "+f"(d[21]), "+f"(d[22]), "+f"(d[23]), "+f"(d[24]), "+f"(d[25]), "+f"(d[26]), "+f"(d[27]), "+f"(d[28]), "+f"(d[29]), "+f"(d[30]), "+f"(d[31]), "+f"(d[32]), "+f"(d[33]), "+f"(d[34]), "+f"(d[35]), "+f"(d[36]), "+f"(d[37]), "+f"(d[38]), "+f"(d[39]), "+f"(d[40]), "+f"(d[41]), "+f"(d[42]), "+f"(d[43]), "+f"(d[44]), "+f"(d[45]), "+f"(d[46]), "+f"(d[47]), "+f"(d[48]), "+f"(d[49]), "+f"(d[50]), "+f"(d[51]), "+f"(d[52]), "+f"(d[53]), "+f"(d[54]), "+f"(d[55]), "+f"(d[56]), "+f"(d[57]), "+f"(d[58]), "+f"(d[59]), "+f"(d[60]), "+f"(d[61]), "+f"(d[62]), "+f"(d[63]), "+f"(d[64]), "+f"(d[65]), "+f"(d[66]), "+f"(d[67]), "+f"(d[68]), "+f"(d[69]), "+f"(d[70]), "+f"(d[71]), "+f"(d[72]), "+f"(d[73]), "+f"(d[74]), "+f"(d[75]), "+f"(d[76]), "+f"(d[77]), "+f"(d[78]), "+f"(d[79]), "+f"(d[80]), "+f"(d[81]), "+f"(d[82]), "+f"(d[83]), "+f"(d[84]), "+f"(d[85]), "+f"(d[86]), "+f"(d[87]), "+f"(d[88]), "+f"(d[89]), "+f"(d[90]), "+f"(d[91]), "+f"(d[92]), "+f"(d[93]), "+f"(d[94]), "+f"(d[95])
               : "l"(da), "l"(db), "r"(scale_d));
}

__device__ __forceinline__ uint64_t make_smem_desc(uint32_t smem_addr, uint32_t lbo_bytes, uint32_t sbo_bytes) {
  uint64_t d = 0;
  d |= (uint64_t)((smem_addr & 0x3FFFF) >> 4);
  d |= (uint64_t)((lbo_bytes >> 4) & 0x3FFF) << 16;
  d |= (uint64_t)((sbo_bytes >> 4) & 0x3FFF) << 32;
  d |= (uint64_t)1 << 62;
  return d;
}

template <typename T, int BN, int MT, int TA, int TB, int STEPS, int LIVE>
__device__ __forceinline__ void mma_kblock(float (&acc)[MT][BN / 2], uint64_t da, uint64_t db, uint32_t a_step, uint32_t b_step) {
  constexpr uint64_t SUB = (uint64_t)(BM * 128) >> 4;
#pragma unroll
  for (int u = 0; u < MT; ++u) acc_fence(acc[u]);
  wgmma_fence();
#pragma unroll
  for (int k = 0; k < STEPS; ++k) {
#pragma unroll
    for (int u = 0; u < LIVE; ++u) {
      if constexpr (Elem<T>::TF32) wgmma(acc[u], da + u * SUB + a_step * k, db + b_step * k, 1u, WgTF32<BN>{});
      else wgmma(acc[u], da + u * SUB + a_step * k, db + b_step * k, 1u, WgBF16<BN, TA, TB>{});
    }
  }
  wgmma_commit();
  wgmma_wait0();
#pragma unroll
  for (int u = 0; u < MT; ++u) acc_fence(acc[u]);
}

template <typename T, int BN, int MT, int TA, int TB, int LIVE>
__device__ __forceinline__ void mma_kblock_steps(float (&acc)[MT][BN / 2], uint64_t da, uint64_t db, uint32_t a_step, uint32_t b_step,
                                                 int steps) {
  static_assert(Elem<T>::BK / Elem<T>::MMA_K == 4, "k-steps per k-block");
  if (steps == 4) mma_kblock<T, BN, MT, TA, TB, 4, LIVE>(acc, da, db, a_step, b_step);
  else if (steps == 3) mma_kblock<T, BN, MT, TA, TB, 3, LIVE>(acc, da, db, a_step, b_step);
  else if (steps == 2) mma_kblock<T, BN, MT, TA, TB, 2, LIVE>(acc, da, db, a_step, b_step);
  else mma_kblock<T, BN, MT, TA, TB, 1, LIVE>(acc, da, db, a_step, b_step);
}
template <typename T, int BN, int MT, int TA, int TB>
__device__ __forceinline__ void mma_kblock_trim(float (&acc)[MT][BN / 2], uint64_t da, uint64_t db, uint32_t a_step, uint32_t b_step,
                                                int steps, int n_live) {
  if (MT == 2 && n_live == 1) mma_kblock_steps<T, BN, MT, TA, TB, 1>(acc, da, db, a_step, b_step, steps);
  else mma_kblock_steps<T, BN, MT, TA, TB, MT>(acc, da, db, a_step, b_step, steps);
}

__device__ __forceinline__ void xpose_tf32(uint8_t* dst, const uint8_t* src, int rows, int tid) {
  for (int c = tid; c < rows * 8; c += 128) {
    const int k = c & 31, mn = (c >> 5) * 4;
    const int mi = mn & 31;
    const float4 v = *reinterpret_cast<const float4*>(src + (mn >> 5) * 4096 + k * 128 + ((((mi >> 2) ^ (k & 7))) << 4));
    const float e[4] = {v.x, v.y, v.z, v.w};
#pragma unroll
    for (int i = 0; i < 4; ++i) {
      const int r = mn + i;
      uint32_t t;
      asm("cvt.rna.tf32.f32 %0, %1;" : "=r"(t) : "f"(e[i]));
      *reinterpret_cast<uint32_t*>(dst + r * 128 + ((((k >> 2) ^ (r & 7))) << 4) + (k & 3) * 4) = t;
    }
  }
}

__device__ __forceinline__ void tile_mn(const Params& p, int rem, int& mti, int& nti) {
  if (p.group_m <= 0) { nti = rem / p.mt; mti = rem - nti * p.mt; return; }
  const int band_sz = p.group_m * p.nt;
  const int band = rem / band_sz, within = rem - band * band_sz;
  const int rows = min(p.group_m, p.mt - band * p.group_m);
  nti = within / rows; mti = band * p.group_m + (within - nti * rows);
}

template <typename OP, int BN, int MT>
__global__ void __launch_bounds__(NUM_THREADS, 1)
gemm_wgmma(const __grid_constant__ CUtensorMap tmap_a0, const __grid_constant__ CUtensorMap tmap_b0,
           const __grid_constant__ CUtensorMap tmap_a1, const __grid_constant__ CUtensorMap tmap_b1, const Params p) {
  using T = typename Operand<OP>::Type;
  constexpr bool SGD = Operand<OP>::kSgd;
  static_assert(!SGD || MT == 1, "the SGD epilogue handles 128-row tiles");
  using C = Cfg<T, BN, MT>;
  using E = Elem<T>;
  constexpr int BK = E::BK, MMA_K = E::MMA_K, ATOM = E::ATOM;
  constexpr int SUB_BYTES = BM * 128;
  constexpr int TM = MT * BM;
  extern __shared__ uint8_t smem_raw[];
  const uint32_t smem_raw_u32 = smem_u32(smem_raw);
  const uint32_t smem_base = (smem_raw_u32 + 1023u) & ~1023u;
  const uint32_t xpose_base = smem_base + C::STAGES * C::STAGE_BYTES;
  const uint32_t staging_base = xpose_base + C::XPOSE_BYTES;
  const uint32_t bar_base = staging_base + C::STAGING_BYTES;
  auto full_bar = [&](int s) { return bar_base + 8u * s; };
  auto empty_bar = [&](int s) { return bar_base + 8u * (C::STAGES + s); };
  auto generic = [&](uint32_t a) { return smem_raw + (a - smem_raw_u32); };

  const int warp = threadIdx.x >> 5;
  const int lane = threadIdx.x & 31;
  const int wg = threadIdx.x >> 7;
  const int num_kb_total = p.num_kb;
  const int tiles_mn = p.mt * p.nt;
  const int per_group = tiles_mn * p.splits;
  const int total_tiles = per_group * p.groups;

  if (threadIdx.x == 0) {
    tma_prefetch_desc(&tmap_a0);
    tma_prefetch_desc(&tmap_b0);
    if (p.groups > 1) { tma_prefetch_desc(&tmap_a1); tma_prefetch_desc(&tmap_b1); }
    for (int s = 0; s < C::STAGES; ++s) { mbar_init(full_bar(s), 1); mbar_init(empty_bar(s), NUM_CONSUMER_WARPS); }
    fence_barrier_init();
  }
  __syncthreads();

  if (wg == 0) {
    asm volatile("setmaxnreg.dec.sync.aligned.u32 %0;" ::"n"(PRODUCER_REGS));
    if (warp != 0) return;
    const bool leader = elect_one();
    const bool skip_a = (p.dbg & 1) != 0, skip_b = (p.dbg & 2) != 0;
    const bool issue_a = leader && !skip_a, issue_b = leader && !skip_b;
    int stage = 0; uint32_t phase = 0;
    for (int tile = blockIdx.x; tile < total_tiles; tile += gridDim.x) {
      const int grp = tile >= per_group ? 1 : 0;
      const int t2 = tile - grp * per_group;
      const CUtensorMap* const tma_a = grp ? &tmap_a1 : &tmap_a0;
      const CUtensorMap* const tma_b = grp ? &tmap_b1 : &tmap_b0;
      const int split = t2 / tiles_mn, rem = t2 - split * tiles_mn;
      int mti, nti;
      tile_mn(p, rem, mti, nti);
      const int m0 = mti * TM, n0 = nti * BN;
      const int kb0 = split * p.kb_per_split, kb1 = min(num_kb_total, kb0 + p.kb_per_split);
      const int n_sub = (MT == 2 && m0 + BM < p.M) ? 2 : 1;
      if (p.conv_mode == 1) {
        const int hw = p.cHo * p.cWo;
        int img0[MT], bw0[MT], bh0[MT];
#pragma unroll
        for (int u = 0; u < MT; ++u) {
          const int mu = m0 + u * BM;
          img0[u] = mu / hw; const int r0_ = mu - img0[u] * hw; const int p0 = r0_ / p.cWo, q0 = r0_ - p0 * p.cWo;
          bw0[u] = q0 * p.cS - p.cP; bh0[u] = p0 * p.cS - p.cP;
        }
        int tap = kb0 / p.c_chunks, cc = kb0 - tap * p.c_chunks;
        int r_ = tap / p.cKW, s_ = tap - r_ * p.cKW;
        const uint32_t tx = (skip_a ? 0u : (uint32_t)(n_sub * SUB_BYTES)) + (skip_b ? 0u : (uint32_t)C::B_BYTES);
        const bool b_t = p.b_mn != 0;
        const int ntaps = p.cKH * p.cKW;
        for (int kb = kb0; kb < kb1; ++kb) {
          mbar_wait(empty_bar(stage), phase ^ 1u);
          const uint32_t sa = smem_base + stage * C::STAGE_BYTES;
          const uint32_t fb = full_bar(stage);
          if (leader) mbar_expect_tx(fb, tx);
          if (issue_a) {
#pragma unroll
            for (int u = 0; u < MT; ++u)
              if (u < n_sub) tma_load_im2col(sa + u * SUB_BYTES, tma_a, fb, cc * BK, bw0[u], bh0[u], img0[u], s_, r_);
          }
          if (issue_b) {
            if (!b_t) {
              tma_load_3d(sa + C::A_BYTES, tma_b, fb, cc * BK, tap, n0);
            } else {
#pragma unroll
              for (int j = 0; j < (BN >= ATOM ? BN / ATOM : 1); ++j)
                tma_load_3d(sa + C::A_BYTES + j * (BK * 128), tma_b, fb, n0 + ATOM * j, ntaps - 1 - tap, cc * BK);
            }
          }
          if (++cc == p.c_chunks) { cc = 0; ++tap; if (++s_ == p.cKW) { s_ = 0; ++r_; } }
          if (++stage == C::STAGES) { stage = 0; phase ^= 1u; }
        }
      } else if (p.conv_mode == 2) {
        constexpr int NBOX = (BN >= ATOM) ? BN / ATOM : 1;
        const int total_boxes = p.cKH * p.cKW * p.c_chunks;
        const int w_box0 = nti * NBOX;
        int bc[NBOX], bs[NBOX], br[NBOX];
        int nbox = 0;
#pragma unroll
        for (int j = 0; j < NBOX; ++j) {
          const int box = w_box0 + j;
          const int tapj = box / p.c_chunks, c64 = box - tapj * p.c_chunks;
          br[j] = tapj / p.cKW; bs[j] = tapj - br[j] * p.cKW; bc[j] = c64 * ATOM;
          if (box < total_boxes) ++nbox;
        }
        if (skip_b) nbox = 0;
        const uint32_t tx = (skip_a ? 0u : (uint32_t)C::A_BYTES) + (uint32_t)(nbox * (BK * 128));
        const int hw = p.cHo * p.cWo;
        int pix = kb0 * BK;
        int img = pix / hw; const int r2 = pix - img * hw; int pp = r2 / p.cWo, qq = r2 - pp * p.cWo;
        for (int kb = kb0; kb < kb1; ++kb) {
          mbar_wait(empty_bar(stage), phase ^ 1u);
          const uint32_t sa = smem_base + stage * C::STAGE_BYTES;
          const uint32_t sb = sa + C::A_BYTES;
          const uint32_t fb = full_bar(stage);
          if (leader) mbar_expect_tx(fb, tx);
          if (issue_a) {
#pragma unroll
            for (int j = 0; j < BM / ATOM; ++j) tma_load_2d(sa + j * (BK * 128), tma_a, fb, m0 + ATOM * j, pix);
          }
          if (issue_b) {
            const int cw = qq * p.cS - p.cP, ch = pp * p.cS - p.cP;
#pragma unroll
            for (int j = 0; j < NBOX; ++j)
              if (j < nbox) tma_load_im2col(sb + j * (BK * 128), tma_b, fb, bc[j], cw, ch, img, bs[j], br[j]);
          }
          pix += BK; qq += BK;
          while (qq >= p.cWo) { qq -= p.cWo; if (++pp == p.cHo) { pp = 0; ++img; } }
          if (++stage == C::STAGES) { stage = 0; phase ^= 1u; }
        }
      } else {
        const uint32_t tx = (skip_a ? 0u : (uint32_t)(n_sub * SUB_BYTES)) + (skip_b ? 0u : (uint32_t)C::B_BYTES);
        const bool a_mn = p.a_mn != 0, b_mn = p.b_mn != 0;
        int k0 = kb0 * BK;
        for (int kb = kb0; kb < kb1; ++kb, k0 += BK) {
          mbar_wait(empty_bar(stage), phase ^ 1u);
          const uint32_t sa = smem_base + stage * C::STAGE_BYTES;
          const uint32_t sb = sa + C::A_BYTES;
          const uint32_t fb = full_bar(stage);
          if (leader) mbar_expect_tx(fb, tx);
          if (issue_a) {
#pragma unroll
            for (int u = 0; u < MT; ++u) {
              if (u < n_sub) {
                if (!a_mn) {
                  tma_load_2d(sa + u * SUB_BYTES, tma_a, fb, k0, m0 + u * BM);
                } else {
#pragma unroll
                  for (int j = 0; j < BM / ATOM; ++j) tma_load_2d(sa + u * SUB_BYTES + j * (BK * 128), tma_a, fb, m0 + u * BM + ATOM * j, k0);
                }
              }
            }
          }
          if (issue_b) {
            if (!b_mn) {
              tma_load_2d(sb, tma_b, fb, k0, n0);
            } else {
#pragma unroll
              for (int j = 0; j < (BN >= ATOM ? BN / ATOM : 1); ++j) tma_load_2d(sb + j * (BK * 128), tma_b, fb, n0 + ATOM * j, k0);
            }
          }
          if (++stage == C::STAGES) { stage = 0; phase ^= 1u; }
        }
      }
    }
    __syncwarp();
    return;
  }

  asm volatile("setmaxnreg.inc.sync.aligned.u32 %0;" ::"n"(CONSUMER_REGS));
  const int cw = wg - 1;
  const int ctid = threadIdx.x & 127;
  const int wi = warp & 3;
  const bool skip_mma = (p.dbg & 4) != 0;
  const bool a_mn = p.a_mn != 0, b_mn = p.b_mn != 0;
  const bool xa = C::XPOSE && a_mn, xb = C::XPOSE && b_mn;
  const uint32_t xa_base = xpose_base + (uint32_t)cw * (C::XA_BYTES + C::B_BYTES), xb_base = xa_base + C::XA_BYTES;
  constexpr uint32_t kMnStep = (uint32_t)(MMA_K * 128) >> 4;
  const uint32_t a_step = (a_mn && !xa) ? kMnStep : 2u, b_step = (b_mn && !xb) ? kMnStep : 2u;
  const uint32_t a_lbo = (a_mn && !xa) ? (uint32_t)(BK * 128) : 16u, b_lbo = (b_mn && !xb) ? (uint32_t)(BK * 128) : 16u;
  const int mode = E::TF32 ? 0 : ((a_mn ? 1 : 0) | (b_mn ? 2 : 0));

  const int esz = p.out_bf16 ? 2 : 4;
  const uint32_t pitch = (uint32_t)(32 * esz + 16);
  uint8_t* const wstage = generic(staging_base) + (size_t)(cw * 4 + wi) * 16 * C::STAGING_ROW;
  const int vec_per_row = (32 * esz) / 16;
  const int rows_per_it = 32 / vec_per_row;
  const int lr = lane / vec_per_row, lv = lane % vec_per_row;
  const bool ld_ok = (((long long)p.ldc * esz) % 16) == 0;
  const int fr = lane >> 2, fc = 2 * (lane & 3);
  constexpr int STEPS = BK / MMA_K;
  const int k_chunks = p.conv_mode == 1 ? p.c_chunks : 1;
  const int tail_steps = p.conv_mode == 1 ? (p.cCg - (p.c_chunks - 1) * BK + MMA_K - 1) / MMA_K : STEPS;
  float acc[MT][BN / 2];
  int stage = 0; uint32_t phase = 0;
  for (int tile = blockIdx.x; tile < total_tiles; tile += gridDim.x) {
    const int grp = tile >= per_group ? 1 : 0;
    const int t2 = tile - grp * per_group;
    const int split = t2 / tiles_mn, rem = t2 - split * tiles_mn;
    int mti, nti;
    tile_mn(p, rem, mti, nti);
    const int m0 = mti * TM, n0 = nti * BN;
    const int kb0 = split * p.kb_per_split, kb1 = min(num_kb_total, kb0 + p.kb_per_split);
    int n_live = 0;
#pragma unroll
    for (int u = 0; u < MT; ++u) n_live += (m0 + u * BM + 64 * cw < p.M) ? 1 : 0;
    int cc = kb0 % k_chunks;
#pragma unroll
    for (int u = 0; u < MT; ++u)
#pragma unroll
      for (int i = 0; i < BN / 2; ++i) acc[u][i] = 0.f;
    for (int kb = kb0; kb < kb1; ++kb) {
      mbar_wait(full_bar(stage), phase);
      const int steps = cc == k_chunks - 1 ? tail_steps : STEPS;
      if (++cc == k_chunks) cc = 0;
      const uint32_t sa = smem_base + stage * C::STAGE_BYTES;
      uint32_t a_addr = sa + (uint32_t)cw * (64 * 128), b_addr = sa + C::A_BYTES;
      if (n_live > 0) {
        if constexpr (C::XPOSE) {
          if (xa || xb) {
            wg_bar(cw);
            if (xa) { xpose_tf32(generic(xa_base), generic(a_addr), 64, ctid); a_addr = xa_base; }
            if (xb) { xpose_tf32(generic(xb_base), generic(b_addr), BN, ctid); b_addr = xb_base; }
            fence_proxy_async();
            wg_bar(cw);
          }
        }
        if (!skip_mma) {
          const uint64_t da = make_smem_desc(a_addr, a_lbo, 1024u), db = make_smem_desc(b_addr, b_lbo, 1024u);
          if (mode == 0) mma_kblock_trim<T, BN, MT, 0, 0>(acc, da, db, a_step, b_step, steps, n_live);
          else if (mode == 1) mma_kblock_trim<T, BN, MT, 1, 0>(acc, da, db, a_step, b_step, steps, n_live);
          else if (mode == 2) mma_kblock_trim<T, BN, MT, 0, 1>(acc, da, db, a_step, b_step, steps, n_live);
          else mma_kblock_trim<T, BN, MT, 1, 1>(acc, da, db, a_step, b_step, steps, n_live);
        }
      }
      __syncwarp();
      if (lane == 0) mbar_arrive(empty_bar(stage));
      if (++stage == C::STAGES) { stage = 0; phase ^= 1u; }
    }

    if constexpr (SGD) {
      const Params::Sgd& s = p.sgd;
      const Hyper h{*s.lr_ptr, s.mu, s.inv_k, s.nesterov};
      const int mbase = m0 + 64 * cw + 16 * wi;
      if (mbase >= p.M) continue;
      constexpr int kPitch = 32 * 4 + 16;
      const int vr = lane >> 3, vc = lane & 7;
      float4 wb[2][4], ub[2][4];
      auto load_wu = [&](int c, float4 (&w)[4], float4 (&u)[4]) {
        const int nb = n0 + 32 * c;
        if (nb + 32 > p.N) return;
#pragma unroll
        for (int it = 0; it < 4; ++it) {
          const long long gm = (long long)mbase + 4 * it + vr;
          if (gm < p.M) {
            const long long e = gm * s.ldw + nb + 4 * vc;
            w[it] = *reinterpret_cast<const float4*>(s.W + e);
            u[it] = *reinterpret_cast<const float4*>(s.U + e);
          }
        }
      };
      load_wu(0, wb[0], ub[0]);
#pragma unroll
      for (int c = 0; c < BN / 32; ++c) {
        const int nb = n0 + 32 * c;
        const bool full = nb + 32 <= p.N;
        if (c + 1 < BN / 32) load_wu(c + 1, wb[(c + 1) & 1], ub[(c + 1) & 1]);
        float4 (&w)[4] = wb[c & 1];
        float4 (&u)[4] = ub[c & 1];
#pragma unroll
        for (int f = 0; f < 4; ++f) {
          const int i = 4 * c + f, j = 8 * f + fc;
          *reinterpret_cast<float2*>(wstage + fr * kPitch + j * 4) =
              make_float2(fmaf(acc[0][4 * i], p.alpha, 0.f), fmaf(acc[0][4 * i + 1], p.alpha, 0.f));
          *reinterpret_cast<float2*>(wstage + (fr + 8) * kPitch + j * 4) =
              make_float2(fmaf(acc[0][4 * i + 2], p.alpha, 0.f), fmaf(acc[0][4 * i + 3], p.alpha, 0.f));
        }
        __syncwarp();
        if (full) {
#pragma unroll
          for (int it = 0; it < 4; ++it) {
            const int rr = 4 * it + vr;
            const long long gm = (long long)mbase + rr;
            if (gm < p.M) {
              const long long e = gm * s.ldw + nb + 4 * vc;
              const float4 g = *reinterpret_cast<const float4*>(wstage + rr * kPitch + vc * 16);
              sgd4(w[it], u[it], g, h, s.lr_mult, s.wd);
              *reinterpret_cast<float4*>(s.W + e) = w[it];
              *reinterpret_cast<float4*>(s.U + e) = u[it];
              if (s.H) *reinterpret_cast<uint2*>(s.H + e) = pack_bf16x4(w[it]);
            }
          }
        } else if (nb < p.N) {
          const int n = nb + lane;
          if (n < p.N) {
            for (int rr = 0; rr < 16; ++rr) {
              const long long gm = (long long)mbase + rr;
              if (gm >= p.M) break;
              const long long e = gm * s.ldw + n;
              float4 w1 = make_float4(s.W[e], 0.f, 0.f, 0.f), u1 = make_float4(s.U[e], 0.f, 0.f, 0.f);
              const float4 g1 = make_float4(*reinterpret_cast<const float*>(wstage + rr * kPitch + lane * 4), 0.f, 0.f, 0.f);
              sgd4(w1, u1, g1, h, s.lr_mult, s.wd);
              s.W[e] = w1.x;
              s.U[e] = u1.x;
              if (s.H) s.H[e] = __float2bfloat16_rn(w1.x);
            }
          }
        }
        __syncwarp();
      }
      continue;
    }

    uint8_t* const Cg_ptr = reinterpret_cast<uint8_t*>(grp ? p.C1 : p.C);
    const float* const bias_ptr = grp ? p.bias1 : p.bias;
#pragma unroll
    for (int u = 0; u < MT; ++u) {
      const int mbase = m0 + u * BM + 64 * cw + 16 * wi;
      if (mbase >= p.M) continue;
      float bm0 = 0.f, bm1 = 0.f;
      if (p.bias_mode == 2) {
        if (mbase + fr < p.M) bm0 = __ldg(bias_ptr + mbase + fr);
        if (mbase + fr + 8 < p.M) bm1 = __ldg(bias_ptr + mbase + fr + 8);
      }
#pragma unroll
      for (int c = 0; c < BN / 32; ++c) {
        const int cc = 32 * c;
        int nb = n0 + cc, n_end_c = p.N;
        if (p.conv_mode == 2) {
          const int box = nti * (BN >= ATOM ? BN / ATOM : 1) + cc / ATOM;
          if (box < p.cKH * p.cKW * p.c_chunks) {
            const int tap = box / p.c_chunks, cch = box - tap * p.c_chunks;
            nb = tap * p.cCg + cch * ATOM + (cc % ATOM);
            n_end_c = tap * p.cCg + min(p.cCg, cch * ATOM + ATOM);
          } else {
            nb = 0; n_end_c = 0;
          }
        }
#pragma unroll
        for (int f = 0; f < 4; ++f) {
          const int i = 4 * c + f;
          const int j = 8 * f + fc;
          float v0 = acc[u][4 * i], v1 = acc[u][4 * i + 1], v2 = acc[u][4 * i + 2], v3 = acc[u][4 * i + 3];
          float b0 = bm0, b1 = bm0, b2 = bm1, b3 = bm1;
          if (p.bias_mode == 1) {
            const int n = nb + j;
            b0 = b2 = (n < n_end_c) ? __ldg(bias_ptr + n) : 0.f;
            b1 = b3 = (n + 1 < n_end_c) ? __ldg(bias_ptr + n + 1) : 0.f;
          }
          v0 = fmaf(v0, p.alpha, b0); v1 = fmaf(v1, p.alpha, b1); v2 = fmaf(v2, p.alpha, b2); v3 = fmaf(v3, p.alpha, b3);
          if (p.relu) { v0 = fmaxf(v0, 0.f); v1 = fmaxf(v1, 0.f); v2 = fmaxf(v2, 0.f); v3 = fmaxf(v3, 0.f); }
          if (p.out_bf16) {
            *reinterpret_cast<__nv_bfloat162*>(wstage + fr * pitch + j * 2) = __floats2bfloat162_rn(v0, v1);
            *reinterpret_cast<__nv_bfloat162*>(wstage + (fr + 8) * pitch + j * 2) = __floats2bfloat162_rn(v2, v3);
          } else {
            *reinterpret_cast<float2*>(wstage + fr * pitch + j * 4) = make_float2(v0, v1);
            *reinterpret_cast<float2*>(wstage + (fr + 8) * pitch + j * 4) = make_float2(v2, v3);
          }
        }
        __syncwarp();
        const bool staged = (nb + 32 <= n_end_c) && ld_ok && (((reinterpret_cast<uintptr_t>(Cg_ptr) + (long long)nb * esz) % 16) == 0);
        if (staged) {
          const int bulk_kind = p.rs_world > 0 ? 4 : (p.atomic_out ? 2 : 1);
          if (p.bulk & bulk_kind) {
            fence_proxy_async();
            const long long gm = (long long)mbase + lane;
            if (lane < 16 && gm < p.M) {
              const uint32_t ssrc = smem_u32(wstage + (size_t)lane * pitch);
              const uint32_t nbytes = (uint32_t)(32 * esz);
              if (p.rs_world > 0) {
                bool local;
                float* d = rs_addr(p, p.rs_e0 + gm * p.ldc + nb, local);
                bulk_reduce_add_f32(d, ssrc, nbytes);
              } else if (p.atomic_out) {
                bulk_reduce_add_f32(Cg_ptr + ((long long)gm * p.ldc + nb) * esz, ssrc, nbytes);
              } else {
                bulk_store(Cg_ptr + ((long long)gm * p.ldc + nb) * esz, ssrc, nbytes);
              }
            }
            bulk_commit();
            bulk_wait_read();
          } else {
            uint8_t* gbase = Cg_ptr + (long long)nb * esz + (long long)lv * 16;
            for (int r0 = 0; r0 < 16; r0 += rows_per_it) {
              const int rr = r0 + lr;
              const long long gm = (long long)mbase + rr;
              if (gm < p.M) {
                const uint4 val = *reinterpret_cast<const uint4*>(wstage + (size_t)rr * pitch + (size_t)lv * 16);
                uint8_t* gp = gbase + gm * p.ldc * esz;
                if (p.rs_world > 0) {
                  bool local;
                  float* d = rs_addr(p, p.rs_e0 + gm * p.ldc + nb + lv * 4, local);
                  if (local) {
                    asm volatile("red.global.add.v4.f32 [%0], {%1, %2, %3, %4};" ::"l"(d), "f"(__uint_as_float(val.x)),
                                 "f"(__uint_as_float(val.y)), "f"(__uint_as_float(val.z)), "f"(__uint_as_float(val.w)) : "memory");
                  } else {
                    asm volatile("red.relaxed.sys.global.add.v4.f32 [%0], {%1, %2, %3, %4};" ::"l"(d), "f"(__uint_as_float(val.x)),
                                 "f"(__uint_as_float(val.y)), "f"(__uint_as_float(val.z)), "f"(__uint_as_float(val.w)) : "memory");
                  }
                } else if (p.atomic_out) {
                  asm volatile("red.global.add.v4.f32 [%0], {%1, %2, %3, %4};" ::"l"(gp), "f"(__uint_as_float(val.x)),
                               "f"(__uint_as_float(val.y)), "f"(__uint_as_float(val.z)), "f"(__uint_as_float(val.w)) : "memory");
                } else {
                  *reinterpret_cast<uint4*>(gp) = val;
                }
              }
            }
          }
        } else if (nb < n_end_c) {
          const int n = nb + lane;
          if (n < n_end_c) {
            for (int rr = 0; rr < 16; ++rr) {
              const long long gm = (long long)mbase + rr;
              if (gm >= p.M) break;
              if (p.out_bf16) {
                reinterpret_cast<__nv_bfloat16*>(Cg_ptr)[gm * p.ldc + n] = *reinterpret_cast<const __nv_bfloat16*>(wstage + rr * pitch + lane * 2);
                continue;
              }
              const float v = *reinterpret_cast<const float*>(wstage + rr * pitch + lane * 4);
              if (p.rs_world > 0) { bool local; red_add_sys_f32(rs_addr(p, p.rs_e0 + gm * p.ldc + n, local), v); }
              else if (p.atomic_out) atomicAdd(reinterpret_cast<float*>(Cg_ptr) + gm * p.ldc + n, v);
              else reinterpret_cast<float*>(Cg_ptr)[gm * p.ldc + n] = v;
            }
          }
        }
        __syncwarp();
      }
    }
  }
  if (p.bulk) bulk_wait_all();
}


typedef CUresult (*PFN_encodeTiled)(CUtensorMap*, CUtensorMapDataType, cuuint32_t, void*, const cuuint64_t*, const cuuint64_t*,
                                    const cuuint32_t*, const cuuint32_t*, CUtensorMapInterleave, CUtensorMapSwizzle,
                                    CUtensorMapL2promotion, CUtensorMapFloatOOBfill);

static PFN_encodeTiled get_encode() {
  static PFN_encodeTiled fn = nullptr;
  static std::once_flag once;
  std::call_once(once, [] {
    void* f = nullptr;
    cudaDriverEntryPointQueryResult q;
    cudaError_t e = cudaGetDriverEntryPoint("cuTensorMapEncodeTiled", &f, cudaEnableDefault, &q);
    if (e == cudaSuccess && q == cudaDriverEntryPointSuccess) fn = (PFN_encodeTiled)f;
    (void)cudaGetLastError();
  });
  if (!fn) throw std::runtime_error("tmpi_native: cuTensorMapEncodeTiled unavailable (no CUDA driver?)");
  return fn;
}

static CUtensorMapDataType f32_map_type() {
  static const bool rnd = [] { const char* e = getenv("TMPI_TF32_TMA_ROUND"); return !(e && e[0] == '0'); }();
  return rnd ? CU_TENSOR_MAP_DATA_TYPE_TFLOAT32 : CU_TENSOR_MAP_DATA_TYPE_FLOAT32;
}

static CUtensorMap make_tmap(const void* ptr, uint64_t inner, uint64_t outer, uint64_t pitch_bytes, uint32_t box_outer, int esz = 2,
                             int mn_major = 0) {
  if ((reinterpret_cast<uintptr_t>(ptr) & 15) != 0) throw std::runtime_error("tmpi_native: TMA operand base must be 16B aligned");
  if ((pitch_bytes & 15) != 0) throw std::runtime_error("tmpi_native: TMA operand row pitch must be a multiple of 16 bytes");
  using Key = std::tuple<const void*, uint64_t, uint64_t, uint64_t, uint32_t, int, int>;
  static std::map<Key, CUtensorMap> cache;
  static std::mutex mu;
  Key key{ptr, inner, outer, pitch_bytes, box_outer, esz, mn_major};
  const CUtensorMapSwizzle swz = CU_TENSOR_MAP_SWIZZLE_128B;
  std::lock_guard<std::mutex> lk(mu);
  auto it = cache.find(key);
  if (it != cache.end()) return it->second;
  CUtensorMap m;
  cuuint64_t dims[2] = {inner, outer};
  cuuint64_t strides[1] = {pitch_bytes};
  cuuint32_t box[2] = {(cuuint32_t)(128 / esz), box_outer};
  cuuint32_t estr[2] = {1u, 1u};
  CUresult r = get_encode()(&m, esz == 4 ? f32_map_type() : CU_TENSOR_MAP_DATA_TYPE_BFLOAT16, 2, const_cast<void*>(ptr), dims, strides, box, estr,
                            CU_TENSOR_MAP_INTERLEAVE_NONE, swz, CU_TENSOR_MAP_L2_PROMOTION_L2_256B,
                            CU_TENSOR_MAP_FLOAT_OOB_FILL_NONE);
  if (r != CUDA_SUCCESS) throw std::runtime_error("tmpi_native: cuTensorMapEncodeTiled failed, code " + std::to_string((int)r));
  if (cache.size() > 4096) cache.clear();
  cache[key] = m;
  return m;
}

extern int g_dbg;
extern int g_bulk;
static int bulk_default() {
  static const int v = [] { const char* e = getenv("TMPI_GEMM_BULK"); return e ? atoi(e) : 4; }();
  return v;
}

template <typename OP, int BN, int MT>
static void launch(const CUtensorMap& ta, const CUtensorMap& tb, Params& p, int splits, cudaStream_t st,
                   const CUtensorMap* ta1 = nullptr, const CUtensorMap* tb1 = nullptr) {
  using T = typename Operand<OP>::Type;
  using C = Cfg<T, BN, MT>;
  p.dbg = g_dbg;
  p.bulk = g_bulk < 0 ? bulk_default() : g_bulk;
  if (!ta1) { p.groups = 1; p.C1 = nullptr; p.bias1 = nullptr; }
  static bool attr_set = false;
  if (!attr_set) {
    check_cuda(cudaFuncSetAttribute(gemm_wgmma<OP, BN, MT>, cudaFuncAttributeMaxDynamicSharedMemorySize, C::SMEM_BYTES), "gemm smem attr");
    attr_set = true;
  }
  if (MT == 2 && sizeof(T) == 4 && (p.a_mn || p.b_mn)) throw std::runtime_error("tmpi_native: 256-row tf32 tiles need K-major operands");
  if (sizeof(T) == 4 && p.out_bf16) throw std::runtime_error("tmpi_native: the tf32 path stores fp32");
  const long long total = (long long)p.mt * p.nt * splits * p.groups;
  const int grid = (int)std::min<long long>(total, (long long)sm_count());
  gemm_wgmma<OP, BN, MT><<<grid, NUM_THREADS, C::SMEM_BYTES, st>>>(ta, tb, ta1 ? *ta1 : ta, tb1 ? *tb1 : tb, p);
  count_launch();
  TMPI_CHECK_LAUNCH("gemm_wgmma"); ::tmpi::check_capture(st, "gemm_wgmma");
}

}
}
```

theanompi_b200/csrc/nn_kernels.cu:

```cuda
#include "common.cuh"
#include "api.h"
#include <algorithm>

namespace tmpi {

static inline int grid_for(long long n, int block) { return (int)((n + block - 1) / block); }

template <int HALF>
__global__ void lrn_fwd_kernel(const __nv_bfloat16* __restrict__ x, __nv_bfloat16* __restrict__ y, long long rows, int C,
                               float k, float alpha, float beta) {
  const int nvec = C >> 3;
  const unsigned idx = blockIdx.x * blockDim.x + threadIdx.x;
  if (idx >= (unsigned)rows * (unsigned)nvec) return;
  const long long r = idx / (unsigned)nvec;
  const int cv = (int)(idx - (unsigned)r * (unsigned)nvec);
  const __nv_bfloat16* row = x + r * C;
  float xs[24];
#pragma unroll
  for (int v = 0; v < 3; ++v) {
    const int c = (cv - 1 + v) * 8;
    if (c >= 0 && c < C) unpack8(*reinterpret_cast<const bf16x8*>(row + c), xs + 8 * v);
    else {
#pragma unroll
      for (int i = 0; i < 8; ++i) xs[8 * v + i] = 0.f;
// ... 1006 lines not shown
            dv[t] = *reinterpret_cast<const bf16x8*>(dyp + o);
          }
        }
      }
      const long long xi = irow + (unsigned)(w * g.C + cv * 8);
      bf16x8 yv;
      if (FUSE) yv = *reinterpret_cast<const bf16x8*>(y + xi);
      float acc[8];
#pragma unroll
      for (int i = 0; i < 8; ++i) acc[i] = 0.f;
#pragma unroll
      for (int t = 0; t < MAXW * MAXW; ++t) {
        if (ok[t]) {
          const uint32_t me4 = me[t] * 0x01010101u;
          const uint32_t eq_lo = __vcmpeq4(av[t].x, me4), eq_hi = __vcmpeq4(av[t].y, me4);
          const uint32_t* dw = reinterpret_cast<const uint32_t*>(&dv[t]);
          const uint32_t w0 = dw[0] & __byte_perm(eq_lo, 0, 0x1100), w1 = dw[1] & __byte_perm(eq_lo, 0, 0x3322);
          const uint32_t w2 = dw[2] & __byte_perm(eq_hi, 0, 0x1100), w3 = dw[3] & __byte_perm(eq_hi, 0, 0x3322);
          acc[0] += __uint_as_float(w0 << 16); acc[1] += __uint_as_float(w0 & 0xFFFF0000u);
          acc[2] += __uint_as_float(w1 << 16); acc[3] += __uint_as_float(w1 & 0xFFFF0000u);
          acc[4] += __uint_as_float(w2 << 16); acc[5] += __uint_as_float(w2 & 0xFFFF0000u);
          acc[6] += __uint_as_float(w3 << 16); acc[7] += __uint_as_float(w3 & 0xFFFF0000u);
        }
      }
      bf16x8 pk = pack8(acc);
      if (FUSE) {
        uint32_t* pw = reinterpret_cast<uint32_t*>(&pk);
        const uint32_t* yw = reinterpret_cast<const uint32_t*>(&yv);
#pragma unroll
        for (int i = 0; i < 4; ++i) pw[i] &= __vcmpgts2(yw[i], 0u);
      }
      *reinterpret_cast<bf16x8*>(dym + xi) = pk;
      if (FUSE) {
        unpack8(pk, acc);
#pragma unroll
        for (int i = 0; i < 8; ++i) tot[i] += acc[i];
      }
    }
  }
  if (!FUSE) return;
  if (tw < RL) {
#pragma unroll
    for (int i = 0; i < 8; ++i) sm[(tw * VT + tv) * 8 + i] = tot[i];
  }
  __syncthreads();
  if (threadIdx.x < VT * 8) {
    const int v = threadIdx.x / 8, i = threadIdx.x % 8;
    const int c = (blockIdx.y * VT + v) * 8 + i;
    if (c < g.C) {
      float sacc = 0.f;
      for (int t = 0; t < RL; ++t) sacc += sm[(t * VT + v) * 8 + i];
      atomicAdd(c < c_split ? db0 + c : db1 + (c - c_split), sacc);
    }
  }
}

void maxpool_relu_bias_bwd(const void* dyp, const void* arg, const void* y, void* dym, void* db0, void* db1, int c_split, int N, int H,
                           int W, int C, int Ho, int Wo, int k, int s, int p, int accumulate, cudaStream_t st) {
  if (C % 8) throw std::runtime_error("maxpool_relu_bias_bwd: C must be a multiple of 8");
  if ((long long)H * W * C >= (1LL << 31)) throw std::runtime_error("maxpool_relu_bias_bwd: image too large for 32-bit in-image offsets");
  PoolGeom g{N, H, W, C, Ho, Wo, k, s, p};
  const int nvec = C / 8;
  const int VT = nvec < 32 ? nvec : 32;
  const int RL = 256 / VT;
  dim3 grid((unsigned)N * H, (unsigned)((nvec + VT - 1) / VT));
  const size_t smem = (size_t)RL * VT * 8 * sizeof(float);
  if (c_split > C) c_split = C;
  if (!accumulate) check_cuda(cudaMemsetAsync(db0, 0, (size_t)c_split * 4, st), "maxpool_relu_bias_bwd memset");
  if (!accumulate && c_split < C) check_cuda(cudaMemsetAsync(db1, 0, (size_t)(C - c_split) * 4, st), "maxpool_relu_bias_bwd memset");
  const int maxw = (k + s - 1) / s;
  auto DYP = (const __nv_bfloat16*)dyp; auto A = (const uint8_t*)arg; auto Y = (const __nv_bfloat16*)y; auto DM = (__nv_bfloat16*)dym;
  if (maxw == 1) maxpool_relu_bias_bwd_kernel<1, true><<<grid, 256, smem, st>>>(DYP, A, Y, DM, (float*)db0, (float*)db1, c_split, g, VT);
  else if (maxw == 2) maxpool_relu_bias_bwd_kernel<2, true><<<grid, 256, smem, st>>>(DYP, A, Y, DM, (float*)db0, (float*)db1, c_split, g, VT);
  else if (maxw == 3) maxpool_relu_bias_bwd_kernel<3, true><<<grid, 256, smem, st>>>(DYP, A, Y, DM, (float*)db0, (float*)db1, c_split, g, VT);
  else throw std::runtime_error("maxpool_relu_bias_bwd: pooling windows overlapping more than 3x3 outputs are not supported");
  count_launch(); TMPI_CHECK_LAUNCH("maxpool_relu_bias_bwd"); ::tmpi::check_capture(st, "maxpool_relu_bias_bwd");
}

struct ConvGeom { int N, H, W, Ctot, c_off, Cg, KH, KW, Ho, Wo, s, p; long long ldcol; int K; };

template <typename T>
__global__ void __launch_bounds__(256) im2col_vec_kernel(const T* __restrict__ x, T* __restrict__ col, ConvGeom g) {
  constexpr int IM2COL_ROWS = 8;
  constexpr int N = VecIO<T>::N;
  const int cvn = g.Cg >> VecIO<T>::LOG2N;
  const int per_m = g.KH * g.KW * cvn;
  const long long M = (long long)g.N * g.Ho * g.Wo;
  const long long m_base = (long long)blockIdx.x * IM2COL_ROWS;
  for (int rr = 0; rr < IM2COL_ROWS; ++rr) {
    const long long m = m_base + rr;
    if (m >= M) return;
    const int wo = (int)(m % g.Wo); const long long t = m / g.Wo;
    const int ho = (int)(t % g.Ho); const int n = (int)(t / g.Ho);
    const int h0 = ho * g.s - g.p, w0 = wo * g.s - g.p;
    const T* xin = x + (long long)n * g.H * g.W * g.Ctot + g.c_off;
    T* dst = col + m * g.ldcol;
    for (int v = threadIdx.x; v < per_m; v += blockDim.x) {
      const int kk = v / cvn, cv = v - kk * cvn;
      const int kh = kk / g.KW, kw = kk - kh * g.KW;
      const int h = h0 + kh, w = w0 + kw;
      typename VecIO<T>::Raw val;
      if (h >= 0 && h < g.H && w >= 0 && w < g.W)
        val = *reinterpret_cast<const typename VecIO<T>::Raw*>(xin + ((long long)h * g.W + w) * g.Ctot + cv * N);
      else {
        const float zero[N] = {};
        val = VecIO<T>::pack(zero);
      }
      *reinterpret_cast<typename VecIO<T>::Raw*>(dst + kk * g.Cg + cv * N) = val;
    }
  }
}

template <typename T>
__global__ void im2col_scalar_kernel(const T* __restrict__ x, T* __restrict__ col, ConvGeom g) {
  const int per_m = g.KH * g.KW + 1;
  long long idx = (long long)blockIdx.x * blockDim.x + threadIdx.x;
  long long M = (long long)g.N * g.Ho * g.Wo;
  if (idx >= M * per_m) return;
  const long long m = idx / per_m; const int kk = (int)(idx % per_m);
  T* dst = col + m * g.ldcol;
  if (kk == g.KH * g.KW) { for (int c = g.K; c < g.ldcol; ++c) dst[c] = from_f<T>(0.f); return; }
  const int kh = kk / g.KW, kw = kk % g.KW;
  const int wo = (int)(m % g.Wo); long long t = m / g.Wo;
  const int ho = (int)(t % g.Ho); const int n = (int)(t / g.Ho);
  const int h = ho * g.s - g.p + kh, w = wo * g.s - g.p + kw;
  const bool ok = (h >= 0 && h < g.H && w >= 0 && w < g.W);
  const T* src = x + (((long long)n * g.H + h) * g.W + w) * g.Ctot + g.c_off;
  dst += (long long)kk * g.Cg;
  for (int c = 0; c < g.Cg; ++c) dst[c] = ok ? src[c] : from_f<T>(0.f);
}

template <typename T>
__global__ void __launch_bounds__(256) im2col_rows_kernel(const T* __restrict__ x, T* __restrict__ col, ConvGeom g) {
  constexpr int N = VecIO<T>::N;
  extern __shared__ __align__(16) unsigned char im2col_smem[];
  T* rows = reinterpret_cast<T*>(im2col_smem);
  const int n = blockIdx.x / g.Ho, ho = blockIdx.x % g.Ho;
  const int rowlen = g.W * g.Cg;
  const bool dense = (g.Cg == g.Ctot);
  for (int kh = 0; kh < g.KH; ++kh) {
    const int h = ho * g.s - g.p + kh;
    T* dst = rows + kh * rowlen;
    if (h < 0 || h >= g.H) {
      for (int e = threadIdx.x; e < rowlen; e += blockDim.x) dst[e] = from_f<T>(0.f);
    } else if (dense) {
      const T* src = x + ((long long)n * g.H + h) * g.W * g.Ctot;
      for (int e = threadIdx.x; e < rowlen; e += blockDim.x) dst[e] = src[e];
    } else {
      const T* src = x + ((long long)n * g.H + h) * g.W * g.Ctot + g.c_off;
      for (int e = threadIdx.x; e < rowlen; e += blockDim.x) { const int w = e / g.Cg; dst[e] = src[(long long)w * g.Ctot + (e - w * g.Cg)]; }
    }
  }
  __syncthreads();
  const int run = g.KW * g.Cg;
  const int vec_per_row = (int)(g.ldcol >> VecIO<T>::LOG2N);
  T* out = col + ((long long)n * g.Ho + ho) * g.Wo * g.ldcol;
  for (int i = threadIdx.x; i < g.Wo * vec_per_row; i += blockDim.x) {
    const int wo = i / vec_per_row, e0 = (i - wo * vec_per_row) * N;
    const int xbase = (wo * g.s - g.p) * g.Cg;
    int kh = e0 / run, r = e0 - kh * run;
    __align__(16) T v[N];
#pragma unroll
    for (int j = 0; j < N; ++j) {
      T t = from_f<T>(0.f);
      if (e0 + j < g.K) {
        const int xi = xbase + r;
        if (xi >= 0 && xi < rowlen) t = rows[kh * rowlen + xi];
      }
      v[j] = t;
      if (++r == run) { r = 0; ++kh; }
    }
    *reinterpret_cast<uint4*>(out + (long long)wo * g.ldcol + e0) = *reinterpret_cast<const uint4*>(v);
  }
}

template <typename T, int ACT, bool BIAS>
__global__ void col2im_vec_kernel(const T* __restrict__ dcol, T* __restrict__ dx, ConvGeom g, const float* __restrict__ bias, float slope,
                                  int c_real) {
  constexpr int N = VecIO<T>::N;
  const unsigned cvn = (unsigned)(g.Cg >> VecIO<T>::LOG2N);
  const unsigned idx = blockIdx.x * blockDim.x + threadIdx.x;
  const unsigned total = (unsigned)g.N * g.H * g.W * cvn;
  if (idx >= total) return;
  const int cv = (int)(idx % cvn); unsigned t = idx / cvn;
  const int w = (int)(t % g.W); t /= g.W;
  const int h = (int)(t % g.H); const int n = (int)(t / g.H);
  float acc[N];
#pragma unroll
  for (int i = 0; i < N; ++i) acc[i] = 0.f;
  for (int kh = 0; kh < g.KH; ++kh) {
    const int th = h + g.p - kh;
    if (th < 0 || th % g.s) continue;
    const int ho = th / g.s;
    if (ho >= g.Ho) continue;
    for (int kw = 0; kw < g.KW; ++kw) {
      const int tw = w + g.p - kw;
      if (tw < 0 || tw % g.s) continue;
      const int wo = tw / g.s;
      if (wo >= g.Wo) continue;
      const long long m = ((long long)n * g.Ho + ho) * g.Wo + wo;
      float v[N];
      VecIO<T>::ld(dcol + m * g.ldcol + (long long)(kh * g.KW + kw) * g.Cg + cv * N, v);
#pragma unroll
      for (int i = 0; i < N; ++i) acc[i] += v[i];
    }
  }
  if (BIAS) {
#pragma unroll
    for (int i = 0; i < N; ++i) acc[i] += __ldg(bias + cv * N + i);
  }
#pragma unroll
  for (int i = 0; i < N; ++i) acc[i] = act_fwd<ACT>(acc[i], slope);
  if (BIAS || ACT != ACT_NONE) {
#pragma unroll
    for (int i = 0; i < N; ++i) if (cv * N + i >= c_real) acc[i] = 0.f;
  }
  VecIO<T>::st(dx + (((long long)n * g.H + h) * g.W + w) * g.Ctot + g.c_off + cv * N, acc);
}

template <typename T>
static void im2col_t(const void* x, void* col, const ConvGeom& g, cudaStream_t st) {
  constexpr int N = VecIO<T>::N;
  const long long M = (long long)g.N * g.Ho * g.Wo;
  if (g.Cg % N == 0 && g.c_off % N == 0 && g.Ctot % N == 0 && g.ldcol == g.K) {
    im2col_vec_kernel<T><<<grid_for(M, 8), 256, 0, st>>>((const T*)x, (T*)col, g);
  } else if (g.ldcol % N == 0 && (size_t)g.KH * g.W * g.Cg * sizeof(T) <= 48 * 1024) {
    im2col_rows_kernel<T><<<g.N * g.Ho, 256, (size_t)g.KH * g.W * g.Cg * sizeof(T), st>>>((const T*)x, (T*)col, g);
  } else {
    const long long total = M * (g.KH * g.KW + 1);
    im2col_scalar_kernel<T><<<grid_for(total, 256), 256, 0, st>>>((const T*)x, (T*)col, g);
  }
}

void im2col(const void* x, void* col, int N, int H, int W, int Ctot, int c_off, int Cg, int KH, int KW, int Ho, int Wo, int s, int p,
            long long ldcol, int f32, cudaStream_t st) {
  ConvGeom g{N, H, W, Ctot, c_off, Cg, KH, KW, Ho, Wo, s, p, ldcol, KH * KW * Cg};
  if (f32) im2col_t<float>(x, col, g, st);
  else im2col_t<__nv_bfloat16>(x, col, g, st);
  count_launch(); TMPI_CHECK_LAUNCH("im2col"); ::tmpi::check_capture(st, "im2col");
}

void col2im(const void* dcol, void* dx, int N, int H, int W, int Ctot, int c_off, int Cg, int KH, int KW, int Ho, int Wo, int s, int p,
            long long ldcol, int f32, cudaStream_t st) {
  const int V = f32 ? 4 : 8;
  if (Cg % V || c_off % V || Ctot % V || ldcol % V)
    throw std::runtime_error(f32 ? "col2im: channel counts must be multiples of 4" : "col2im: channel counts must be multiples of 8");
  ConvGeom g{N, H, W, Ctot, c_off, Cg, KH, KW, Ho, Wo, s, p, ldcol, KH * KW * Cg};
  long long total = (long long)N * H * W * (Cg / V);
  if (total >= (1LL << 32)) throw std::runtime_error("col2im: tensor too large for 32-bit indexing");
  if (f32) col2im_vec_kernel<float, ACT_NONE, false><<<grid_for(total, 256), 256, 0, st>>>((const float*)dcol, (float*)dx, g, nullptr, 0.f, 0);
  else col2im_vec_kernel<__nv_bfloat16, ACT_NONE, false><<<grid_for(total, 256), 256, 0, st>>>((const __nv_bfloat16*)dcol, (__nv_bfloat16*)dx, g,
                                                                                               nullptr, 0.f, 0);
  count_launch(); TMPI_CHECK_LAUNCH("col2im"); ::tmpi::check_capture(st, "col2im");
}

template <typename T>
static void col2im_bias_act_t(const void* dcol, void* y, const ConvGeom& g, const float* bias, int act, float slope, int c_real,
                              long long total, cudaStream_t st) {
  const int gr = grid_for(total, 256);
  auto D = (const T*)dcol; auto Y = (T*)y;
#define C2I(A) (bias ? col2im_vec_kernel<T, A, true><<<gr, 256, 0, st>>>(D, Y, g, bias, slope, c_real) \
                     : col2im_vec_kernel<T, A, false><<<gr, 256, 0, st>>>(D, Y, g, bias, slope, c_real))
  if (act == ACT_NONE) C2I(ACT_NONE);
  else if (act == ACT_RELU) C2I(ACT_RELU);
  else if (act == ACT_LEAKY) C2I(ACT_LEAKY);
  else if (act == ACT_SIGMOID) C2I(ACT_SIGMOID);
  else throw std::runtime_error("col2im_bias_act: unknown activation");
#undef C2I
}
void col2im_bias_act(const void* dcol, void* y, const float* bias, int N, int H, int W, int C, int KH, int KW, int Hi, int Wi, int s, int p,
                     long long ldcol, int act, float slope, int c_real, int f32, cudaStream_t st) {
  const int V = f32 ? 4 : 8;
  if (C % V || ldcol % V) throw std::runtime_error(f32 ? "col2im_bias_act: channel counts must be multiples of 4"
                                                       : "col2im_bias_act: channel counts must be multiples of 8");
  ConvGeom g{N, H, W, C, 0, C, KH, KW, Hi, Wi, s, p, ldcol, KH * KW * C};
  const long long total = (long long)N * H * W * (C / V);
  if (total >= (1LL << 32)) throw std::runtime_error("col2im_bias_act: tensor too large for 32-bit indexing");
  if (act == ACT_NONE && !bias && c_real < C) throw std::runtime_error("col2im_bias_act: padded channels need a bias or an activation");
  if (f32) col2im_bias_act_t<float>(dcol, y, g, bias, act, slope, c_real, total, st);
  else col2im_bias_act_t<__nv_bfloat16>(dcol, y, g, bias, act, slope, c_real, total, st);
  count_launch(); TMPI_CHECK_LAUNCH("col2im_bias_act"); ::tmpi::check_capture(st, "col2im_bias_act");
}

template <typename T>
__global__ void pad_rows_kernel(const T* __restrict__ src, T* __restrict__ dst, long long rows, int cols, long long src_ld, long long dst_ld) {
  long long idx = (long long)blockIdx.x * blockDim.x + threadIdx.x;
  if (idx >= rows * dst_ld) return;
  const long long r = idx / dst_ld; const int c = (int)(idx % dst_ld);
  dst[idx] = c < cols ? src[r * src_ld + c] : from_f<T>(0.f);
}
void pad_rows(const void* src, void* dst, long long rows, int cols, long long src_ld, long long dst_ld, int f32, cudaStream_t st) {
  if (f32) pad_rows_kernel<float><<<grid_for(rows * dst_ld, 256), 256, 0, st>>>((const float*)src, (float*)dst, rows, cols, src_ld, dst_ld);
  else pad_rows_kernel<__nv_bfloat16><<<grid_for(rows * dst_ld, 256), 256, 0, st>>>((const __nv_bfloat16*)src, (__nv_bfloat16*)dst, rows, cols,
                                                                                      src_ld, dst_ld);
  count_launch(); TMPI_CHECK_LAUNCH("pad_rows"); ::tmpi::check_capture(st, "pad_rows");
}

template <int SCT>
__global__ void __launch_bounds__(256) space_to_depth_kernel(const __nv_bfloat16* __restrict__ x, __nv_bfloat16* __restrict__ y, int N, int H,
                                                             int W, int C, int S, int Hs, int Ws, int Cp, int P) {
  const int i = blockIdx.x % Hs, n = blockIdx.x / Hs;
  const int SC = SCT > 0 ? SCT : S * C;
  const int WC = W * C;
  const int cp = threadIdx.x;
  const int dy = cp / SC, e = cp - dy * SC;
  const int h = i * S + dy - P;
  const bool chan_ok = cp < S * SC && h >= 0 && h < H;
  __nv_bfloat16* orow = y + ((long long)n * Hs + i) * Ws * Cp + cp;
  const __nv_bfloat16* irow = x + ((long long)n * H + (chan_ok ? h : 0)) * WC;
  const __nv_bfloat16 zero = f_to_bf16(0.f);
  const int shift = e - P * C;
  for (int j = threadIdx.y; j < Ws; j += blockDim.y) {
    const int col = j * SC + shift;
    orow[(unsigned)(j * Cp)] = (chan_ok && col >= 0 && col < WC) ? irow[col] : zero;
  }
}
__global__ void space_to_depth_f32_kernel(const float* __restrict__ x, float* __restrict__ y, int N, int H, int W, int C, int S, int Hs, int Ws,
                                          int Cp, int P) {
  const long long idx = (long long)blockIdx.x * blockDim.x + threadIdx.x;
  const long long total = (long long)N * Hs * Ws * Cp;
  if (idx >= total) return;
  const int cp = (int)(idx % Cp); long long t = idx / Cp;
  const int j = (int)(t % Ws); t /= Ws;
  const int i = (int)(t % Hs); const int n = (int)(t / Hs);
  float v = 0.f;
  if (cp < S * S * C) {
    const int c = cp % C, d = cp / C, dy = d / S, dx = d % S;
    const int h = i * S + dy - P, w = j * S + dx - P;
    if (h >= 0 && h < H && w >= 0 && w < W) v = x[(((long long)n * H + h) * W + w) * C + c];
  }
  y[idx] = v;
}

void space_to_depth(const void* x, void* y, int N, int H, int W, int C, int S, int Hs, int Ws, int Cp, int P, int f32, cudaStream_t st) {
  if (f32) {
    space_to_depth_f32_kernel<<<grid_for((long long)N * Hs * Ws * Cp, 256), 256, 0, st>>>((const float*)x, (float*)y, N, H, W, C, S, Hs, Ws, Cp, P);
    count_launch(); TMPI_CHECK_LAUNCH("space_to_depth"); ::tmpi::check_capture(st, "space_to_depth");
    return;
  }
  if (Cp > 256) throw std::runtime_error("space_to_depth: more than 256 packed channels");
  const dim3 blk((unsigned)Cp, (unsigned)std::max(1, 256 / Cp));
  auto X = (const __nv_bfloat16*)x; auto Y = (__nv_bfloat16*)y;
  if (S * C == 12) space_to_depth_kernel<12><<<(unsigned)N * Hs, blk, 0, st>>>(X, Y, N, H, W, C, S, Hs, Ws, Cp, P);
  else space_to_depth_kernel<0><<<(unsigned)N * Hs, blk, 0, st>>>(X, Y, N, H, W, C, S, Hs, Ws, Cp, P);
  count_launch(); TMPI_CHECK_LAUNCH("space_to_depth"); ::tmpi::check_capture(st, "space_to_depth");
}

template <typename T>
__global__ void s2d_filter_kernel(const void* __restrict__ src, void* __restrict__ dst, int O, int KH, int KW, int C, int S, int KHs, int KWs,
                                  int Cp, int dir) {
  if (dir == 0) {
    const int total = O * KHs * KWs * Cp;
    for (int i = blockIdx.x * blockDim.x + threadIdx.x; i < total; i += gridDim.x * blockDim.x) {
      const int cp = i % Cp; int t = i / Cp;
      const int b = t % KWs; t /= KWs;
      const int a = t % KHs; const int o = t / KHs;
      T v = from_f<T>(0.f);
      if (cp < S * S * C) {
        const int c = cp % C, d = cp / C, dy = d / S, dx = d % S;
        const int kh = a * S + dy, kw = b * S + dx;
        if (kh < KH && kw < KW) v = reinterpret_cast<const T*>(src)[(((long long)o * KH + kh) * KW + kw) * C + c];
      }
      reinterpret_cast<T*>(dst)[i] = v;
    }
  } else {
    const int total = O * KH * KW * C;
    for (int i = blockIdx.x * blockDim.x + threadIdx.x; i < total; i += gridDim.x * blockDim.x) {
      const int c = i % C; int t = i / C;
      const int kw = t % KW; t /= KW;
      const int kh = t % KH; const int o = t / KH;
      const int a = kh / S, dy = kh % S, b = kw / S, dx = kw % S;
      const float v = reinterpret_cast<const float*>(src)[(((long long)o * KHs + a) * KWs + b) * Cp + (dy * S + dx) * C + c];
      if (dir == 2) reinterpret_cast<float*>(dst)[i] += v;
      else reinterpret_cast<float*>(dst)[i] = v;
    }
  }
}
void s2d_filter(const void* src, void* dst, int O, int KH, int KW, int C, int S, int KHs, int KWs, int Cp, int dir, int f32, cudaStream_t st) {
  const int total = dir == 0 ? O * KHs * KWs * Cp : O * KH * KW * C;
  const int grid = std::min(grid_for(total, 256), sm_count() * 8);
  if (f32) s2d_filter_kernel<float><<<grid, 256, 0, st>>>(src, dst, O, KH, KW, C, S, KHs, KWs, Cp, dir);
  else s2d_filter_kernel<__nv_bfloat16><<<grid, 256, 0, st>>>(src, dst, O, KH, KW, C, S, KHs, KWs, Cp, dir);
  count_launch(); TMPI_CHECK_LAUNCH("s2d_filter"); ::tmpi::check_capture(st, "s2d_filter");
}

template <typename Tin, typename Tout>
__global__ void __launch_bounds__(128) crop_mirror_norm_kernel(const Tin* __restrict__ x, const float* __restrict__ mean, int mean_mode,
                                        float scale, const float* __restrict__ cscale, Tout* __restrict__ out, const int* __restrict__ offs,
                                        const uint8_t* __restrict__ flips, int N, int H, int W, int C, int ch, int cw, int Cout) {
  const int ox = blockIdx.y * blockDim.x + threadIdx.x;
  if (ox >= cw) return;
  const int oy = blockIdx.x % ch, n = blockIdx.x / ch;
  const int sy = offs[2 * n] + oy;
  const int sx = offs[2 * n + 1] + (flips[n] ? (cw - 1 - ox) : ox);
  const unsigned pix = (unsigned)(sy * W + sx) * (unsigned)C;
  const Tin* src = x + (long long)n * H * W * C + pix;
  const float* mp = mean_mode == 2 ? mean + pix : mean;
  Tout* o = out + ((long long)blockIdx.x * cw + ox) * Cout;
  if (C == 3 && Cout == 3) {
    const float m0 = mean_mode == 0 ? mp[0] : mp[0], m1 = mean_mode == 0 ? mp[0] : mp[1], m2 = mean_mode == 0 ? mp[0] : mp[2];
    const float s0 = cscale ? scale * cscale[0] : scale, s1 = cscale ? scale * cscale[1] : scale, s2 = cscale ? scale * cscale[2] : scale;
    const float v0 = ((float)src[0] - m0) * s0, v1 = ((float)src[1] - m1) * s1, v2 = ((float)src[2] - m2) * s2;
    o[0] = (Tout)v0; o[1] = (Tout)v1; o[2] = (Tout)v2;
    return;
  }
  for (int c = 0; c < Cout; ++c) {
    float v = 0.f;
    if (c < C) {
      const float m = mean_mode == 0 ? mp[0] : mp[c];
      v = ((float)src[c] - m) * (cscale ? scale * cscale[c] : scale);
    }
    o[c] = (Tout)v;
  }
}

void crop_mirror_norm(const void* x, int in_kind , const void* mean, int mean_mode, float scale, const void* cscale, void* out,
                      int out_bf16, const void* offs, const void* flips, int N, int H, int W, int C, int ch, int cw, int Cout, cudaStream_t st) {
  if ((long long)H * W * C >= (1LL << 31) || (long long)N * ch >= (1LL << 31)) throw std::runtime_error("crop_mirror_norm: image too large");
  const dim3 g((unsigned)(N * ch), (unsigned)((cw + 127) / 128));
  auto M = (const float*)mean; auto O = (const int*)offs; auto F = (const uint8_t*)flips;
#define CMN(TI, TO) crop_mirror_norm_kernel<TI, TO><<<g, 128, 0, st>>>((const TI*)x, M, mean_mode, scale, (const float*)cscale, (TO*)out, O, F, N, H, W, C, ch, cw, Cout)
  if (in_kind == 0) { if (out_bf16) CMN(uint8_t, __nv_bfloat16); else CMN(uint8_t, float); }
  else if (in_kind == 1) { if (out_bf16) CMN(__nv_bfloat16, __nv_bfloat16); else CMN(__nv_bfloat16, float); }
  else { if (out_bf16) CMN(float, __nv_bfloat16); else CMN(float, float); }
#undef CMN
  count_launch(); TMPI_CHECK_LAUNCH("crop_mirror_norm"); ::tmpi::check_capture(st, "crop_mirror_norm");
}

__device__ __forceinline__ void rrc_axis(int o, float ratio, int L, int& i0, int& i1, float& lam) {
  const float s = fmaxf(__fmaf_rn(ratio, (float)o + 0.5f, -0.5f), 0.f);
  i0 = min((int)s, L - 1);
  i1 = i0 + (i0 < L - 1 ? 1 : 0);
  lam = fminf(fmaxf(s - (float)i0, 0.f), 1.f);
}

template <typename Tout>
__global__ void __launch_bounds__(128) resized_crop_mirror_norm_kernel(const uint8_t* __restrict__ x, const float* __restrict__ mean,
                                        int mean_mode, float scale, const float* __restrict__ cscale, Tout* __restrict__ out,
                                        const int4* __restrict__ boxes, const uint8_t* __restrict__ flips, int H, int W, int C, int ch,
                                        int cw) {
  const int ox = blockIdx.y * blockDim.x + threadIdx.x;
  if (ox >= cw) return;
  const int oy = blockIdx.x % ch, n = blockIdx.x / ch;
  const int4 b = boxes[n];
  int iy0, iy1, ix0, ix1;
  float ly, lx;
  rrc_axis(oy, __fdiv_rn((float)b.z, (float)ch), b.z, iy0, iy1, ly);
  rrc_axis(flips[n] ? cw - 1 - ox : ox, __fdiv_rn((float)b.w, (float)cw), b.w, ix0, ix1, lx);
  const unsigned r0 = (unsigned)((b.x + iy0) * W + b.y) * (unsigned)C, r1 = (unsigned)((b.x + iy1) * W + b.y) * (unsigned)C;
  const unsigned c0 = (unsigned)ix0 * (unsigned)C, c1 = (unsigned)ix1 * (unsigned)C;
  const unsigned t00 = r0 + c0, t01 = r0 + c1, t10 = r1 + c0, t11 = r1 + c1;
  const uint8_t* src = x + (long long)n * H * W * C;
  const float wy0 = 1.f - ly, wx0 = 1.f - lx;
  Tout* o = out + ((long long)blockIdx.x * cw + ox) * C;
  auto tap = [&](unsigned t, int c, float s) {
    const float m = mean_mode == 0 ? mean[0] : (mean_mode == 1 ? mean[c] : mean[t + c]);
    return ((float)src[t + c] - m) * s;
  };
  auto blend = [&](int c, float s) {
    return wy0 * (wx0 * tap(t00, c, s) + lx * tap(t01, c, s)) + ly * (wx0 * tap(t10, c, s) + lx * tap(t11, c, s));
  };
  if (C == 3) {
    const float s0 = cscale ? scale * cscale[0] : scale, s1 = cscale ? scale * cscale[1] : scale, s2 = cscale ? scale * cscale[2] : scale;
    const float v0 = blend(0, s0), v1 = blend(1, s1), v2 = blend(2, s2);
    o[0] = (Tout)v0; o[1] = (Tout)v1; o[2] = (Tout)v2;
    return;
  }
  for (int c = 0; c < C; ++c) o[c] = (Tout)blend(c, cscale ? scale * cscale[c] : scale);
}

void resized_crop_mirror_norm(const void* x, const void* mean, int mean_mode, float scale, const void* cscale, void* out, int out_bf16,
                              const void* boxes, const void* flips, int N, int H, int W, int C, int ch, int cw, cudaStream_t st) {
  if ((long long)H * W * C >= (1LL << 31) || (long long)N * ch >= (1LL << 31)) throw std::runtime_error("resized_crop_mirror_norm: image too large");
  const dim3 g((unsigned)(N * ch), (unsigned)((cw + 127) / 128));
  auto X = (const uint8_t*)x; auto M = (const float*)mean; auto CS = (const float*)cscale;
  auto B = (const int4*)boxes; auto F = (const uint8_t*)flips;
  if (out_bf16) resized_crop_mirror_norm_kernel<__nv_bfloat16><<<g, 128, 0, st>>>(X, M, mean_mode, scale, CS, (__nv_bfloat16*)out, B, F, H, W, C, ch, cw);
  else resized_crop_mirror_norm_kernel<float><<<g, 128, 0, st>>>(X, M, mean_mode, scale, CS, (float*)out, B, F, H, W, C, ch, cw);
  count_launch(); TMPI_CHECK_LAUNCH("resized_crop_mirror_norm"); ::tmpi::check_capture(st, "resized_crop_mirror_norm");
}

}
```

Baseline: 0.1075 s/5120img.

## Add dense 48-column dgrad tile with 32B-swizzle B atoms; vectorize space_to_depth

Adds a conv dgrad route for channel counts that are multiples of 16 but not 64. It uses a BN=48 wgmma m64n48 tile with 16-element B atoms loaded via a 32B-swizzled tensor map, so fewer padded columns are computed. The route is taken only when the cost model predicts lower cost and no extra work. The epilogue is generalized to partial 32-column chunks. Separately, space_to_depth now writes 16-byte packed vectors per thread instead of scalar stores, which adds alignment requirements on Cp and the output pointer.

```diff
diff --git a/theanompi_b200/csrc/api.h b/theanompi_b200/csrc/api.h
--- a/theanompi_b200/csrc/api.h
+++ b/theanompi_b200/csrc/api.h
@@ -51,6 +51,7 @@
 int gemm_plan_splits(int tiles, int num_kb, int sms);
 int gemm_plan_tall(long long M, int nt, int out_bf16, int sms);
 std::tuple<int, int, int> gemm_plan_conv(int kind, long long M, int N, int groups, int num_kb, int tall_ok, int sms);
+std::tuple<int, int, int, int> gemm_route_dgrad(long long M, int C, int groups, int num_kb, int tall_ok, int sms);
 void gemm(const void* A, const void* B, void* C, const float* bias, int M, int N, int K, long long lda, long long ldb, long long ldc,
           int a_mn, int b_mn, int out_bf16, int bias_mode, int relu, float alpha, int bn_hint, int splitk, int f32, cudaStream_t st,
           int accumulate = 0);
diff --git a/theanompi_b200/csrc/binding.cpp b/theanompi_b200/csrc/binding.cpp
--- a/theanompi_b200/csrc/binding.cpp
+++ b/theanompi_b200/csrc/binding.cpp
@@ -49,6 +49,7 @@
   m.def("gemm_plan_splits", &gemm_plan_splits);
   m.def("gemm_plan_tall", &gemm_plan_tall);
   m.def("gemm_plan_conv", &gemm_plan_conv);
+  m.def("gemm_route_dgrad", &gemm_route_dgrad);
   m.def("gemm", [](ptr_t A, ptr_t B, ptr_t C, ptr_t bias, int M, int N, int K, long long lda, long long ldb, long long ldc, int a_mn, int b_mn,
                    int out_bf16, int bias_mode, int relu, float alpha, int bn_hint, int splitk, int f32, ptr_t st, int accumulate) {
     gemm(P(A), P(B), P(C), (const float*)P(bias), M, N, K, lda, ldb, ldc, a_mn, b_mn, out_bf16, bias_mode, relu, alpha, bn_hint, splitk, f32,
diff --git a/theanompi_b200/csrc/gemm_wgmma.cu b/theanompi_b200/csrc/gemm_wgmma.cu
--- a/theanompi_b200/csrc/gemm_wgmma.cu
+++ b/theanompi_b200/csrc/gemm_wgmma.cu
@@ -34,15 +34,15 @@
   return w2 * 17 <= w1 * 10;
 }
 
-struct ConvTile { int bn, mt, splits; };
+struct ConvTile { int bn, mt, splits; long long cost, work; };
 static ConvTile choose_conv_tile(int kind, long long M, int N, int groups, int num_kb, int tall_ok, int sms) {
-  static const int kCand[7][2] = {{128, 2}, {128, 1}, {192, 1}, {96, 2}, {96, 1}, {64, 2}, {64, 1}};
+  static const int kCand[8][3] = {{128, 2, 0}, {128, 1, 0}, {192, 1, 0}, {96, 2, 0}, {96, 1, 0}, {64, 2, 0}, {64, 1, 0}, {48, 2, 1}};
   const int kTileOverheadKb = 4, kKblockCols = 64;
   const int kWideWgradMinKb = 1024;
-  ConvTile best{0, 0, 1};
-  long long best_cost = -1;
+  ConvTile best{0, 0, 1, -1, 0};
   for (const auto& c : kCand) {
     const int bn = c[0], mt = c[1];
+    if ((kind == 3) != (c[2] != 0)) continue;
     if (bn == 96 && kind != 0) continue;
     if (kind == 2 && (bn == 64 || mt == 2)) continue;
     if (kind == 2 && bn == 192 && num_kb < kWideWgradMinKb) continue;
@@ -54,9 +54,18 @@
     splits = (num_kb + kb_per - 1) / kb_per;
     const long long waves = (tiles * splits + sms - 1) / sms;
     const long long cost = waves * (kb_per + kTileOverheadKb) * (mt * bn + kKblockCols);
-    if (best_cost < 0 || cost < best_cost) { best_cost = cost; best = {bn, mt, splits}; }
+    if (best.cost < 0 || cost < best.cost) best = {bn, mt, splits, cost, waves * kb_per * mt * bn};
   }
   return best;
+}
+
+struct ConvRoute { ConvTile tile; bool dense; };
+static ConvRoute route_dgrad(long long M, int C, int groups, int num_kb, int tall_ok, int sms) {
+  const ConvTile base = choose_conv_tile(1, M, C, groups, num_kb, tall_ok, sms);
+  if (C % 16 != 0 || C % 64 == 0) return {base, false};
+  const ConvTile dense = choose_conv_tile(3, M, C, groups, num_kb, tall_ok, sms);
+  if (dense.bn != 0 && dense.cost < base.cost && dense.work <= base.work) return {dense, true};
+  return {base, false};
 }
 
 }
@@ -114,6 +123,10 @@
 std::tuple<int, int, int> gemm_plan_conv(int kind, long long M, int N, int groups, int num_kb, int tall_ok, int sms) {
   const wgmma::ConvTile t = wgmma::choose_conv_tile(kind, M, N, groups, num_kb, tall_ok, sms);
   return {t.bn, t.mt, t.splits};
+}
+std::tuple<int, int, int, int> gemm_route_dgrad(long long M, int C, int groups, int num_kb, int tall_ok, int sms) {
+  const wgmma::ConvRoute r = wgmma::route_dgrad(M, C, groups, num_kb, tall_ok, sms);
+  return {r.tile.bn, r.tile.mt, r.tile.splits, r.dense ? 1 : 0};
 }
 
 namespace wgmma {
@@ -234,7 +247,7 @@
   static std::map<Key, CUtensorMap> cache;
   static std::mutex mu;
   Key key{w, O, taps, Cg, box_o, box_c, esz, mn_major};
-  const CUtensorMapSwizzle swz = CU_TENSOR_MAP_SWIZZLE_128B;
+  const CUtensorMapSwizzle swz = box_c * esz == 32 ? CU_TENSOR_MAP_SWIZZLE_32B : CU_TENSOR_MAP_SWIZZLE_128B;
   std::lock_guard<std::mutex> lk(mu);
   auto it = cache.find(key);
   if (it != cache.end()) return it->second;
@@ -263,7 +276,10 @@
   if (M >= (1LL << 31)) throw std::runtime_error("conv_fprop: too many output pixels");
   if (ESZ == 4) out_bf16 = 0;
   const int c_chunks = (Cg + BK - 1) / BK, num_kb = KH * KW * c_chunks;
-  const ConvTile tile = choose_conv_tile(dgrad ? 1 : 0, M, O, ngroups, num_kb, ESZ == 2 ? out_bf16 : !dgrad, sm_count());
+  const int tall_ok = ESZ == 2 ? out_bf16 : !dgrad;
+  const ConvRoute route = (ESZ == 2 && dgrad) ? route_dgrad(M, O, ngroups, num_kb, tall_ok, sm_count())
+                                             : ConvRoute{choose_conv_tile(dgrad ? 1 : 0, M, O, ngroups, num_kb, tall_ok, sm_count()), false};
+  const ConvTile tile = route.tile;
   const int BN = tile.bn;
   const bool tall = tile.mt == 2;
   Params p;
@@ -280,10 +296,13 @@
   CUtensorMap ta[2], tb[2];
   for (int g = 0; g < ngroups; ++g) {
     ta[g] = make_im2col_map(x, N, H, W, Ctot, c_off[g], Cg, KH, KW, S, P, BM, ESZ, 0);
-    tb[g] = dgrad ? make_weight_map(w[g], Cg, KH * KW, O, BK, ATOM, ESZ, 1) : make_weight_map(w[g], O, KH * KW, Cg, BN, BK, ESZ, 0);
+    tb[g] = dgrad ? make_weight_map(w[g], Cg, KH * KW, O, BK, route.dense ? 16 : ATOM, ESZ, 1) : make_weight_map(w[g], O, KH * KW, Cg, BN, BK, ESZ, 0);
   }
   const CUtensorMap* a1 = ngroups > 1 ? &ta[1] : nullptr;
   const CUtensorMap* b1 = ngroups > 1 ? &tb[1] : nullptr;
+  if constexpr (ESZ == 2) {
+    if (route.dense) { launch<T, 48, 2, true>(ta[0], tb[0], p, 1, st, a1, b1); return; }
+  }
   if (tall) {
     if (BN == 128) launch<T, 128, 2>(ta[0], tb[0], p, 1, st, a1, b1);
     else if (BN == 96) launch<T, 96, 2>(ta[0], tb[0], p, 1, st, a1, b1);
diff --git a/theanompi_b200/csrc/gemm_wgmma.cuh b/theanompi_b200/csrc/gemm_wgmma.cuh
--- a/theanompi_b200/csrc/gemm_wgmma.cuh
+++ b/theanompi_b200/csrc/gemm_wgmma.cuh
@@ -239,6 +239,14 @@
                : "l"(da), "l"(db), "r"(scale_d), "n"(TA), "n"(TB));
 }
 
+template <int TA, int TB>
+__device__ __forceinline__ void wgmma(float (&d)[24], uint64_t da, uint64_t db, uint32_t scale_d, WgBF16<48, TA, TB>) {
+  asm volatile("{\n\t.reg .pred p;\n\tsetp.ne.b32 p, %26, 0;\n\t"
+               "wgmma.mma_async.sync.aligned.m64n48k16.f32.bf16.bf16 {%0, %1, %2, %3, %4, %5, %6, %7, %8, %9, %10, %11, %12, %13, %14, %15, %16, %17, %18, %19, %20, %21, %22, %23}, %24, %25, p, 1, 1, %27, %28;\n\t}"
+               : "+f"(d[0]), "+f"(d[1]), "+f"(d[2]), "+f"(d[3]), "+f"(d[4]), "+f"(d[5]), "+f"(d[6]), "+f"(d[7]), "+f"(d[8]), "+f"(d[9]), "+f"(d[10]), "+f"(d[11]), "+f"(d[12]), "+f"(d[13]), "+f"(d[14]), "+f"(d[15]), "+f"(d[16]), "+f"(d[17]), "+f"(d[18]), "+f"(d[19]), "+f"(d[20]), "+f"(d[21]), "+f"(d[22]), "+f"(d[23])
+               : "l"(da), "l"(db), "r"(scale_d), "n"(TA), "n"(TB));
+}
+
 __device__ __forceinline__ void wgmma(float (&d)[48], uint64_t da, uint64_t db, uint32_t scale_d, WgTF32<96>) {
   asm volatile("{\n\t.reg .pred p;\n\tsetp.ne.b32 p, %50, 0;\n\t"
                "wgmma.mma_async.sync.aligned.m64n96k8.f32.tf32.tf32 {%0, %1, %2, %3, %4, %5, %6, %7, %8, %9, %10, %11, %12, %13, %14, %15, %16, %17, %18, %19, %20, %21, %22, %23, %24, %25, %26, %27, %28, %29, %30, %31, %32, %33, %34, %35, %36, %37, %38, %39, %40, %41, %42, %43, %44, %45, %46, %47}, %48, %49, p, 1, 1;\n\t}"
@@ -253,12 +261,12 @@
                : "l"(da), "l"(db), "r"(scale_d));
 }
 
-__device__ __forceinline__ uint64_t make_smem_desc(uint32_t smem_addr, uint32_t lbo_bytes, uint32_t sbo_bytes) {
+__device__ __forceinline__ uint64_t make_smem_desc(uint32_t smem_addr, uint32_t lbo_bytes, uint32_t sbo_bytes, uint32_t layout = 1) {
   uint64_t d = 0;
   d |= (uint64_t)((smem_addr & 0x3FFFF) >> 4);
   d |= (uint64_t)((lbo_bytes >> 4) & 0x3FFF) << 16;
   d |= (uint64_t)((sbo_bytes >> 4) & 0x3FFF) << 32;
-  d |= (uint64_t)1 << 62;
+  d |= (uint64_t)layout << 62;
   return d;
 }
 
@@ -322,16 +330,20 @@
   nti = within / rows; mti = band * p.group_m + (within - nti * rows);
 }
 
-template <typename OP, int BN, int MT>
+template <typename OP, int BN, int MT, bool DENSE = false>
 __global__ void __launch_bounds__(NUM_THREADS, 1)
 gemm_wgmma(const __grid_constant__ CUtensorMap tmap_a0, const __grid_constant__ CUtensorMap tmap_b0,
            const __grid_constant__ CUtensorMap tmap_a1, const __grid_constant__ CUtensorMap tmap_b1, const Params p) {
   using T = typename Operand<OP>::Type;
   constexpr bool SGD = Operand<OP>::kSgd;
   static_assert(!SGD || MT == 1, "the SGD epilogue handles 128-row tiles");
+  static_assert(!SGD || BN % 32 == 0, "the SGD epilogue moves whole 32-column chunks");
   using C = Cfg<T, BN, MT>;
   using E = Elem<T>;
   constexpr int BK = E::BK, MMA_K = E::MMA_K, ATOM = E::ATOM;
+  static_assert(!DENSE || (!E::TF32 && !SGD && BN % 16 == 0), "16-element B atoms: bf16 conv dgrad");
+  constexpr int BATOM = DENSE ? 16 : ATOM;
+  constexpr int BBOX = BK * BATOM * E::ESZ;
   constexpr int SUB_BYTES = BM * 128;
   constexpr int TM = MT * BM;
   extern __shared__ uint8_t smem_raw[];
@@ -408,8 +420,8 @@
               tma_load_3d(sa + C::A_BYTES, tma_b, fb, cc * BK, tap, n0);
             } else {
 #pragma unroll
-              for (int j = 0; j < (BN >= ATOM ? BN / ATOM : 1); ++j)
-                tma_load_3d(sa + C::A_BYTES + j * (BK * 128), tma_b, fb, n0 + ATOM * j, ntaps - 1 - tap, cc * BK);
+              for (int j = 0; j < (BN >= BATOM ? BN / BATOM : 1); ++j)
+                tma_load_3d(sa + C::A_BYTES + j * BBOX, tma_b, fb, n0 + BATOM * j, ntaps - 1 - tap, cc * BK);
             }
           }
           if (++cc == p.c_chunks) { cc = 0; ++tap; if (++s_ == p.cKW) { s_ = 0; ++r_; } }
@@ -501,7 +513,8 @@
   const bool xa = C::XPOSE && a_mn, xb = C::XPOSE && b_mn;
   const uint32_t xa_base = xpose_base + (uint32_t)cw * (C::XA_BYTES + C::B_BYTES), xb_base = xa_base + C::XA_BYTES;
   constexpr uint32_t kMnStep = (uint32_t)(MMA_K * 128) >> 4;
-  const uint32_t a_step = (a_mn && !xa) ? kMnStep : 2u, b_step = (b_mn && !xb) ? kMnStep : 2u;
+  constexpr uint32_t kMnStep16 = (uint32_t)(MMA_K * 32) >> 4;
+  const uint32_t a_step = (a_mn && !xa) ? kMnStep : 2u, b_step = DENSE ? kMnStep16 : ((b_mn && !xb) ? kMnStep : 2u);
   const uint32_t a_lbo = (a_mn && !xa) ? (uint32_t)(BK * 128) : 16u, b_lbo = (b_mn && !xb) ? (uint32_t)(BK * 128) : 16u;
   const int mode = E::TF32 ? 0 : ((a_mn ? 1 : 0) | (b_mn ? 2 : 0));
 
@@ -551,7 +564,8 @@
           }
         }
         if (!skip_mma) {
-          const uint64_t da = make_smem_desc(a_addr, a_lbo, 1024u), db = make_smem_desc(b_addr, b_lbo, 1024u);
+          const uint64_t da = make_smem_desc(a_addr, a_lbo, 1024u);
+          const uint64_t db = DENSE ? make_smem_desc(b_addr, BBOX, 256u, 3u) : make_smem_desc(b_addr, b_lbo, 1024u);
           if (mode == 0) mma_kblock_trim<T, BN, MT, 0, 0>(acc, da, db, a_step, b_step, steps, n_live);
           else if (mode == 1) mma_kblock_trim<T, BN, MT, 1, 0>(acc, da, db, a_step, b_step, steps, n_live);
           else if (mode == 2) mma_kblock_trim<T, BN, MT, 0, 1>(acc, da, db, a_step, b_step, steps, n_live);
@@ -648,8 +662,9 @@
         if (mbase + fr + 8 < p.M) bm1 = __ldg(bias_ptr + mbase + fr + 8);
       }
 #pragma unroll
-      for (int c = 0; c < BN / 32; ++c) {
+      for (int c = 0; c < (BN + 31) / 32; ++c) {
         const int cc = 32 * c;
+        const int ccols = (BN % 32 != 0 && c == BN / 32) ? BN % 32 : 32;
         int nb = n0 + cc, n_end_c = p.N;
         if (p.conv_mode == 2) {
           const int box = nti * (BN >= ATOM ? BN / ATOM : 1) + cc / ATOM;
@@ -663,6 +678,7 @@
         }
 #pragma unroll
         for (int f = 0; f < 4; ++f) {
+          if (8 * f >= ccols) break;
           const int i = 4 * c + f;
           const int j = 8 * f + fc;
           float v0 = acc[u][4 * i], v1 = acc[u][4 * i + 1], v2 = acc[u][4 * i + 2], v3 = acc[u][4 * i + 3];
@@ -683,7 +699,7 @@
           }
         }
         __syncwarp();
-        const bool staged = (nb + 32 <= n_end_c) && ld_ok && (((reinterpret_cast<uintptr_t>(Cg_ptr) + (long long)nb * esz) % 16) == 0);
+        const bool staged = (nb + ccols <= n_end_c) && ld_ok && (((reinterpret_cast<uintptr_t>(Cg_ptr) + (long long)nb * esz) % 16) == 0);
         if (staged) {
           const int bulk_kind = p.rs_world > 0 ? 4 : (p.atomic_out ? 2 : 1);
           if (p.bulk & bulk_kind) {
@@ -691,7 +707,7 @@
             const long long gm = (long long)mbase + lane;
             if (lane < 16 && gm < p.M) {
               const uint32_t ssrc = smem_u32(wstage + (size_t)lane * pitch);
-              const uint32_t nbytes = (uint32_t)(32 * esz);
+              const uint32_t nbytes = (uint32_t)(ccols * esz);
               if (p.rs_world > 0) {
                 bool local;
                 float* d = rs_addr(p, p.rs_e0 + gm * p.ldc + nb, local);
@@ -709,7 +725,7 @@
             for (int r0 = 0; r0 < 16; r0 += rows_per_it) {
               const int rr = r0 + lr;
               const long long gm = (long long)mbase + rr;
-              if (gm < p.M) {
+              if (gm < p.M && (ccols == 32 || lv * 16 < ccols * esz)) {
                 const uint4 val = *reinterpret_cast<const uint4*>(wstage + (size_t)rr * pitch + (size_t)lv * 16);
                 uint8_t* gp = gbase + gm * p.ldc * esz;
                 if (p.rs_world > 0) {
@@ -733,7 +749,7 @@
           }
         } else if (nb < n_end_c) {
           const int n = nb + lane;
-          if (n < n_end_c) {
+          if (n < n_end_c && (ccols == 32 || lane < ccols)) {
             for (int rr = 0; rr < 16; ++rr) {
               const long long gm = (long long)mbase + rr;
               if (gm >= p.M) break;
@@ -812,7 +828,7 @@
   return v;
 }
 
-template <typename OP, int BN, int MT>
+template <typename OP, int BN, int MT, bool DENSE = false>
 static void launch(const CUtensorMap& ta, const CUtensorMap& tb, Params& p, int splits, cudaStream_t st,
                    const CUtensorMap* ta1 = nullptr, const CUtensorMap* tb1 = nullptr) {
   using T = typename Operand<OP>::Type;
@@ -822,14 +838,14 @@
   if (!ta1) { p.groups = 1; p.C1 = nullptr; p.bias1 = nullptr; }
   static bool attr_set = false;
   if (!attr_set) {
-    check_cuda(cudaFuncSetAttribute(gemm_wgmma<OP, BN, MT>, cudaFuncAttributeMaxDynamicSharedMemorySize, C::SMEM_BYTES), "gemm smem attr");
+    check_cuda(cudaFuncSetAttribute(gemm_wgmma<OP, BN, MT, DENSE>, cudaFuncAttributeMaxDynamicSharedMemorySize, C::SMEM_BYTES), "gemm smem attr");
     attr_set = true;
   }
   if (MT == 2 && sizeof(T) == 4 && (p.a_mn || p.b_mn)) throw std::runtime_error("tmpi_native: 256-row tf32 tiles need K-major operands");
   if (sizeof(T) == 4 && p.out_bf16) throw std::runtime_error("tmpi_native: the tf32 path stores fp32");
   const long long total = (long long)p.mt * p.nt * splits * p.groups;
   const int grid = (int)std::min<long long>(total, (long long)sm_count());
-  gemm_wgmma<OP, BN, MT><<<grid, NUM_THREADS, C::SMEM_BYTES, st>>>(ta, tb, ta1 ? *ta1 : ta, tb1 ? *tb1 : tb, p);
+  gemm_wgmma<OP, BN, MT, DENSE><<<grid, NUM_THREADS, C::SMEM_BYTES, st>>>(ta, tb, ta1 ? *ta1 : ta, tb1 ? *tb1 : tb, p);
   count_launch();
   TMPI_CHECK_LAUNCH("gemm_wgmma"); ::tmpi::check_capture(st, "gemm_wgmma");
 }
diff --git a/theanompi_b200/csrc/nn_kernels.cu b/theanompi_b200/csrc/nn_kernels.cu
--- a/theanompi_b200/csrc/nn_kernels.cu
+++ b/theanompi_b200/csrc/nn_kernels.cu
@@ -1332,17 +1332,25 @@
   const int i = blockIdx.x % Hs, n = blockIdx.x / Hs;
   const int SC = SCT > 0 ? SCT : S * C;
   const int WC = W * C;
-  const int cp = threadIdx.x;
-  const int dy = cp / SC, e = cp - dy * SC;
-  const int h = i * S + dy - P;
-  const bool chan_ok = cp < S * SC && h >= 0 && h < H;
-  __nv_bfloat16* orow = y + ((long long)n * Hs + i) * Ws * Cp + cp;
-  const __nv_bfloat16* irow = x + ((long long)n * H + (chan_ok ? h : 0)) * WC;
-  const __nv_bfloat16 zero = f_to_bf16(0.f);
-  const int shift = e - P * C;
-  for (int j = threadIdx.y; j < Ws; j += blockDim.y) {
-    const int col = j * SC + shift;
-    orow[(unsigned)(j * Cp)] = (chan_ok && col >= 0 && col < WC) ? irow[col] : zero;
+  const int nv = Cp >> 3;
+  const __nv_bfloat16* img = x + (long long)n * H * WC;
+  __nv_bfloat16* orow = y + ((long long)n * Hs + i) * Ws * Cp;
+  const unsigned short zero = 0;
+  for (int t = threadIdx.x; t < Ws * nv; t += blockDim.x) {
+    const int j = t / nv, cp0 = (t - j * nv) * 8;
+    uint32_t packed[4];
+#pragma unroll
+    for (int q = 0; q < 8; ++q) {
+      const int cp = cp0 + q;
+      const int dy = cp / SC, e = cp - dy * SC;
+      const int h = i * S + dy - P;
+      const int col = j * SC + e - P * C;
+      unsigned short v = zero;
+      if (cp < S * SC && h >= 0 && h < H && col >= 0 && col < WC)
+        v = __bfloat16_as_ushort(img[(unsigned)(h * WC + col)]);
+      if (q & 1) packed[q >> 1] |= (uint32_t)v << 16; else packed[q >> 1] = v;
+    }
+    *reinterpret_cast<uint4*>(orow + (unsigned)(j * Cp + cp0)) = make_uint4(packed[0], packed[1], packed[2], packed[3]);
   }
 }
 __global__ void space_to_depth_f32_kernel(const float* __restrict__ x, float* __restrict__ y, int N, int H, int W, int C, int S, int Hs, int Ws,
@@ -1368,8 +1376,9 @@
     count_launch(); TMPI_CHECK_LAUNCH("space_to_depth"); ::tmpi::check_capture(st, "space_to_depth");
     return;
   }
-  if (Cp > 256) throw std::runtime_error("space_to_depth: more than 256 packed channels");
-  const dim3 blk((unsigned)Cp, (unsigned)std::max(1, 256 / Cp));
+  if (Cp % 8 || (reinterpret_cast<uintptr_t>(y) & 15)) throw std::runtime_error("space_to_depth: Cp must be a multiple of 8, y 16-byte aligned");
+  if ((long long)H * W * C >= (1LL << 31)) throw std::runtime_error("space_to_depth: image too large for 32-bit in-image offsets");
+  const int blk = 256;
   auto X = (const __nv_bfloat16*)x; auto Y = (__nv_bfloat16*)y;
   if (S * C == 12) space_to_depth_kernel<12><<<(unsigned)N * Hs, blk, 0, st>>>(X, Y, N, H, W, C, S, Hs, Ws, Cp, P);
   else space_to_depth_kernel<0><<<(unsigned)N * Hs, blk, 0, st>>>(X, Y, N, H, W, C, S, Hs, Ws, Cp, P);
```

After: 0.1060 s/5120img, median of 6. 1.01x faster.
